# Kotstantinovskiy/SonicDiffusionBayesLab

Measured on AMD Instinct MI355X. Metric: 512x512 images/sec at 50 DDIM steps, higher is better.
Workload: dtype bf16; 1 GPU; SD-1.5 512x512 DDIM 50 steps, CFG 7.5, batch=8/GPU (BASELINE configs[1]); global_batch=8, sample_size=64, parallelism=batch-shard x1, weights=SD-1.5-shaped synthetic seed 1234

## Files before the change

include/sd_hip.h:

```cpp
#ifndef SD_HIP_H
#define SD_HIP_H

#ifdef __cplusplus
extern "C" {
#endif

typedef struct sd_unet sd_unet;

typedef struct sd_unet_config {
    int sample_size;
    int in_channels;
    int out_channels;
    int num_levels;
    int block_out_channels[8];
    int layers_per_block;
    int attn_levels[8];
    int cross_attention_dim;
    int num_heads;
    int norm_num_groups;
    float norm_eps;
    int context_len;
    int weight_dtype;
    float fp8_act_scale_norm;
    float fp8_act_scale_ff;
// ... 106 lines not shown
int sd_clip_encode(sd_clip* c, void* stream, const int* input_ids, int batch, float* hidden_out, void* workspace,
                   long long workspace_bytes);

typedef struct sd_clip_vision_config {
    int hidden_size;
    int num_layers;
    int num_heads;
    int intermediate_size;
    int image_size;
    int patch_size;
    int projection_dim;
    float layer_norm_eps;
    int hidden_act;
} sd_clip_vision_config;
enum { SD_ACT_QUICK_GELU = 0, SD_ACT_GELU = 1 };
typedef struct sd_unet sd_clip_vision;
int sd_clip_create_projected(const sd_clip_config* cfg, int projection_dim, int eos_token_id, sd_clip** out);
long long sd_clip_text_embeds_workspace_bytes(sd_clip* c, int batch);
int sd_clip_text_embeds(sd_clip* c, void* stream, const int* input_ids, int batch, float* text_embeds, void* workspace,
                        long long workspace_bytes);
int sd_clip_vision_create(const sd_clip_vision_config* cfg, sd_clip_vision** out);
long long sd_clip_vision_workspace_bytes(sd_clip_vision* v, int batch, int height, int width);
int sd_clip_vision_encode(sd_clip_vision* v, void* stream, const unsigned char* images, int batch, int height, int width,
                          float* image_embeds, void* workspace, long long workspace_bytes);
int sd_clip_score(void* stream, const float* image_embeds, const float* text_embeds, int batch, int dim, float* raw,
                  float* score);
typedef struct sd_image_reward_config {
    int vision_hidden_size;
    int vision_num_layers;
    int vision_num_heads;
    int vision_intermediate_size;
    int image_size;
    int patch_size;
    float vision_layer_norm_eps;
    int vocab_size;
    int hidden_size;
    int num_layers;
    int num_heads;
    int intermediate_size;
    int max_positions;
    float layer_norm_eps;
    int hidden_act;
    int position_embedding_absolute;
    int max_text_len;
    float reward_mean, reward_std;
} sd_image_reward_config;
typedef struct sd_unet sd_image_reward;
int sd_image_reward_create(const sd_image_reward_config* cfg, sd_image_reward** out);
long long sd_image_reward_workspace_bytes(sd_image_reward* m, int batch, int height, int width);
int sd_image_reward_score(sd_image_reward* m, void* stream, const unsigned char* images, const int* input_ids,
                          const int* attention_mask, int batch, int text_len, int height, int width, float* rewards,
                          float* features_or_null, void* workspace, long long workspace_bytes);
int sd_clip_resize_taps(int in_size, int out_size, int first, int count, int* xmin, int* xcnt, int* coeffs);

typedef struct sd_inception sd_inception;
int sd_inception_create(sd_inception** out);
void sd_inception_destroy(sd_inception* h);
int sd_inception_num_convs(const sd_inception* h);
int sd_inception_conv_info(const sd_inception* h, int index, char* name, int name_cap, long long shape[4]);
int sd_inception_load_conv(sd_inception* h, const char* name, const float* weight_oihw, long long weight_numel,
                           const float* bias, int cout);
int sd_inception_finalize(sd_inception* h);
long long sd_inception_workspace_bytes(sd_inception* h, int batch, int tap);
int sd_inception_features(sd_inception* h, void* stream, const unsigned char* images, int batch, int height, int width,
                          int tap, float* features, void* workspace, long long workspace_bytes);
int sd_fid_accumulate(void* stream, const float* features, int batch, int dim, double* sum, double* cov_sum,
                      long long* count);
int sd_op_inception_conv(void* stream, const void* X, const void* W, const float* bias, void* Y, int B, int Hin, int Win,
                         int Cin, int Cout, int kh, int kw, int stride, int pad_h, int pad_w, int ldy, int coff, int relu);
int sd_op_maxpool3x3(void* stream, const void* X, void* Y, int B, int H, int W, int C, int stride, int pad, int ldy, int coff);
int sd_op_avgpool3x3(void* stream, const void* X, void* Y, int B, int H, int W, int C, int ldy, int coff);
int sd_op_global_mean(void* stream, const void* X, float* out, int B, int HW, int C);
int sd_op_inception_resize(void* stream, const unsigned char* images, int B, int H, int W, void* out, int out_fp32);

#define SD_PROFILE_KINDS 32
int sd_unet_forward_profiled(sd_unet* u, void* stream, const float* latents, int latent_batch, int unet_batch,
                             float timestep, float* eps_out, void* workspace, long long workspace_bytes, int cache_mode,
                             int cache_branch_id, double kind_ms[SD_PROFILE_KINDS], long long kind_launches[SD_PROFILE_KINDS],
                             double kind_flops[SD_PROFILE_KINDS], double kind_bytes[SD_PROFILE_KINDS]);

long long sd_unet_forward_op_times(sd_unet* u, void* stream, const float* latents, int latent_batch, int unet_batch,
                                   float timestep, float* eps_out, void* workspace, long long workspace_bytes, int cache_mode,
                                   int cache_branch_id, char* text, long long cap);

int sd_unet_debug_tensor(sd_unet* u, void* stream, const char* name, float* host_out, long long numel,
                         void* workspace, int unet_batch, int cache_branch_id);

int sd_sched_step(void* stream, const float* eps, int cfg, float guidance, const float* x, const float* m1,
                  const float* m2, const float* m3, const float* noise, float* prev, float* y2, float* m_out,
                  const float coef[10], long long n);

int sd_cfg_rescale_factors(void* stream, const float* eps, int batch, long long n_per_sample, float guidance,
                           float rescale, float* k_out);
int sd_sched_step_rescaled(void* stream, const float* eps, int cfg, float guidance, const float* x, const float* m1,
                           const float* m2, const float* m3, const float* noise, float* prev, float* y2, float* m_out,
                           const float coef[10], long long n, const float* k, long long n_per_sample);

int sd_sched_step_inpaint(void* stream, const float* eps, int cfg, float guidance, const float* x, const float* m1,
                          const float* m2, const float* m3, const float* noise, float* prev, float* y2, float* m_out,
                          const float coef[10], long long n, const float* k, long long n_per_sample, const float* init,
                          const float* blend_noise, const float* mask, float a, float s, long long hw);
int sd_inpaint_prepare(void* stream, const float* image, const float* mask, float* masked_image, float* latent_mask,
                       int batch, int height, int width);

int sd_op_gemm(void* stream, const void* X, long long ldx, const void* X2, long long ldx2, int K1, const void* W,
               const float* bias, const float* bias2, const void* R, long long ldr, void* C, long long ldc, int M,
               int N, int K, int epi);
int sd_op_gemm_tile_rows(int M, int N, int K);
int sd_op_gemm_splitk(int M, int N, int K, int dtype);
int sd_op_gemm_batched(void* stream, const void* X, long long ldx, const void* W, long long w_batch_stride,
                       int rows_per_batch, const float* bias, const void* R, long long ldr, void* C, long long ldc,
                       int M, int N, int K, int epi, int sm_valid);
int sd_op_gemm_batched_softmax_ln(void* stream, const void* X, long long ldx, const void* W, long long w_batch_stride,
                                  int rows_per_batch, void* C, long long ldc, int M, int N, int K, int sm_valid,
                                  const float* rowstats, int parts, const float* c1, const float* c2, float eps);
int sd_op_conv3x3(void* stream, const void* X, const void* W, const float* bias, const float* bias2, const void* R,
                  void* Y, int B, int Hin, int Win, int Cin, int Cout, int stride, int upsample);
int sd_op_conv3x3_shortcut(void* stream, const void* X, const void* W, const float* bias, const void* Xs1, int Cs1,
                           const void* Xs2, int Cs2, const void* Wsc, void* Y, int B, int H, int Wd, int Cin, int Cout);
int sd_op_conv3x3_shortcut_groupnorm(void* stream, const void* X, const void* W, const float* bias, const void* Xs1, int Cs1,
                                     const void* Xs2, int Cs2, const void* Wsc, void* Y, int B, int H, int Wd, int Cin,
                                     int Cout, const float* gamma, const float* beta, void* Yn, int groups, float eps, int silu);
int sd_op_conv3x3_down_asym(void* stream, const void* X, const void* W, const float* bias, void* Y, int B, int Hin, int Win,
                            int Cin, int Cout);
int sd_op_conv3x3_kernel(int M, int N, int Cin, int Hin, int Win, int stride, int upsample, int dtype);
int sd_op_softmax_rows(void* stream, void* S, long long rows, int cols, float scale);
int sd_op_conv3x3_upsample_subpixel(void* stream, const void* X, const void* W4, const float* bias, void* Y, int B, int Hin,
                                    int Win, int Cin, int Cout);
int sd_op_conv3x3_upsample_subpixel_groupnorm(void* stream, const void* X, const void* W4, const float* bias, void* Y, int B,
                                              int Hin, int Win, int Cin, int Cout, const float* gamma, const float* beta,
                                              void* Yn, int groups, float eps, int silu);
int sd_op_groupnorm(void* stream, const void* x1, int C1, const void* x2, int C2, const float* gamma,
                    const float* beta, void* y, int B, int HW, int groups, float eps, int silu);
int sd_op_conv3x3_groupnorm(void* stream, const void* X, const void* W, const float* bias, const float* bias2,
                            const void* R, void* Y, int B, int Hin, int Win, int Cin, int Cout, const float* gamma,
                            const float* beta, void* Yn, int groups, float eps, int silu);
int sd_op_conv3x3_splitk(int M, int Cout, int Cin, int Hin, int Win, int stride, int upsample);
int sd_op_layernorm(void* stream, const void* x, const float* gamma, const float* beta, void* y, int rows, int C,
                    float eps);
int sd_op_tome_match(void* stream, const void* x, const unsigned char* choice, int B, int h, int w, int C, float* node_max,
                     int* node_idx, int* tok);
int sd_op_tome_select(void* stream, const float* node_max, const int* node_idx, int B, int num_src, int r, int* kept, int* merged,
                      int* dst_idx);
int sd_op_tome_merge(void* stream, const void* x, const int* tok, const int* kept, const int* merged, const int* dst_idx, void* out,
                     long long ldo, int B, int h, int w, int C, int r);
int sd_op_tome_unmerge(void* stream, const void* y, long long ldy, const void* residual, const int* tok, const int* kept,
                       const int* merged, const int* dst_idx, void* out, int B, int h, int w, int C, int r);
int sd_op_attention(void* stream, const void* Q, long long ldq, const void* K, long long ldk, const void* V,
                    long long ldv, void* O, long long ldo, int B, int heads, int Nq, int Nk, int D, float scale);
int sd_op_gemm_qkv_headmajor(void* stream, const void* X, long long ldx, const void* W, void* Q, void* KV, int M, int C,
                             int tokens, int K);
int sd_op_attention_headmajor(void* stream, const void* Q, long long ldq, const void* K, const void* V, void* O,
                              long long ldo, int B, int heads, int Nq, int Nk, int D, float scale);
int sd_op_clip_attention(void* stream, const void* qkv, void* out, int B, int L, int H, int heads);
int sd_op_vit_attention(void* stream, const void* qkv, void* out, int B, int L, int H, int heads);
int sd_op_bert_attention(void* stream, const void* q, long long ldq, const void* k, const void* v, long long ldkv,
                         const int* mask, void* out, long long ldo, int B, int heads, int Lq, int Lk);
int sd_op_reward_head(void* stream, const void* hidden, long long row_stride, const float* w, const float* bias, float mean,
                      float std, int B, int H, float* rewards, float* features);
int sd_op_clip_preprocess(void* stream, const unsigned char* images, int B, int H, int W, int S, int P, unsigned char* crop,
                          void* patches);
int sd_op_conv_in(void* stream, const float* x, int Bsrc, const float* Wt, const float* bias, void* y, int B, int H,
                  int W, int Cin, int Cout);
int sd_op_conv_in_cond(void* stream, const float* x, int Bsrc, const float* cond, int Bcond, const float* Wt,
                       const float* bias, void* y, int B, int H, int W, int Cout);
int sd_op_conv_in_add(void* stream, const float* x, int Bsrc, const void* addend, int Badd, const float* Wt, const float* bias,
                      void* y, int B, int H, int W, int Cout);
int sd_op_residual_add(void* stream, void* x, const long long* dst_off, const void* r, const long long* src_off,
                       const long long* count, int nseg, float scale);
int sd_op_conv_out(void* stream, const void* x, const void* Wp, const float* bias, float* y, int B, int H, int W,
                   int Cin, int Cout);
int sd_op_time_embedding(void* stream, float t, const void* W1, const float* b1, const void* W2, const float* b2,
                         float* scratch, float* temb, int dim_in, int dim);
int sd_op_timestep_cond(void* stream, float t, const float* cond, const void* Wc, float* row, float* emb, int cond_dim,
                        int dim);

int sd_op_ln_partials(int kind, int M, int N);
int sd_op_gemm_rowstats(void* stream, const void* X, long long ldx, const void* W, const float* bias, const void* R,
                        long long ldr, void* C, long long ldc, int M, int N, int K, float* rowstats);
int sd_op_gemm_ln(void* stream, const void* X, long long ldx, const void* Wg, const float* c1, const float* c2,
                  const float* rowstats, int parts, float eps, void* C, long long ldc, int M, int N, int K, int epi);
int sd_op_gemm_plan(void* stream, const void* X, long long ldx, const void* X2, long long ldx2, int K1, const void* W,
                    const float* bias, const float* bias2, const void* R, long long ldr, void* C, long long ldc, int M, int N,
                    int K, float* rowstats, float* stats, const float* ln_rs, int ln_parts, const float* ln_c1, float ln_eps,
                    void* KV, int hm_tokens);
int sd_op_xattn_fused_rowstats(void* stream, const void* X, const void* R, void* Y, const void* At, const void* Bw,
                               const float* bias, int M, int C, int rows_per_sample, int L, float* rowstats);
int sd_op_ip_xattn(void* stream, const void* R, void* Rout, const void* A, const void* Bt, const float* gamma, const float* beta,
                   float eps, long long M, int C, int rows_per_sample, int heads, int T);
int sd_op_xattn_fused(void* stream, const void* X, const void* R, void* Y, const void* At, const void* Bw,
                      const float* bias, int M, int C, int rows_per_sample, int L);
int sd_op_xattn_fused_ln(void* stream, const void* X, const void* R, void* Y, const void* At, const void* Bw,
                         const float* bias, int M, int C, int rows_per_sample, int L, const float* ln_rowstats, int ln_parts,
                         long long ln_rows, const float* c2, float eps, float* rowstats);
int sd_op_conv3x3_ablate(void* stream, const void* X, const void* W, void* Y, int B, int Hin, int Win, int Cin, int Cout,
                         int ablate);
int sd_op_xattn_fused_stamps(void* stream, const void* X, const void* R, void* Y, const void* At, const void* Bw,
                             const float* bias, int M, int C, int rows_per_sample, int L, unsigned long long* stamps);

int sd_op_gemm_fp8(void* stream, const void* X, long long ldx, const void* W, const float* wscale, float xscale,
                   const float* bias, const void* R, long long ldr, void* C, long long ldc, int M, int N, int K, int epi,
                   int out_fp8, float oscale);
int sd_op_conv3x3_fp8(void* stream, const void* X, const void* W, const float* wscale, float xscale, const float* bias,
                      const float* bias2, const void* R, void* Y, int B, int Hin, int Win, int Cin, int Cout, int stride,
                      int upsample);
int sd_op_groupnorm_fp8(void* stream, const void* x1, int C1, const void* x2, int C2, const float* gamma,
                        const float* beta, void* y, int B, int HW, int groups, float eps, int silu, int Cpad, float oscale);
int sd_op_layernorm_fp8(void* stream, const void* x, const float* gamma, const float* beta, void* y, int rows, int C,
                        int Cpad, float eps, float oscale);
int sd_op_quantize_fp8(void* stream, const void* x_bf16, void* y_fp8, long long rows, int C, int Cpad, float scale);
int sd_op_amax_e4m3(void* stream, const void* codes, long long nbytes, unsigned* out_code);

#ifdef __cplusplus
}
#endif
#endif
```

sonicdiffusionbayeslab_amd/_lib.py:

```python
from __future__ import annotations

import ctypes as C
import os
import re
from typing import Optional

HERE = os.path.dirname(os.path.abspath(__file__))
LIB_PATH = os.environ.get("SD_AMD_LIB", os.path.join(HERE, "lib", "libsdhip.so"))
HEADER_PATH = os.path.normpath(os.path.join(HERE, "..", "include", "sd_hip.h"))

ABLATE_LIB_PATH = os.path.join(HERE, "lib", "libsdhip_ablate.so")

_lib: Optional[C.CDLL] = None
_ablate: Optional[C.CDLL] = None


class SdUnetConfig(C.Structure):
    _fields_ = [
        ("sample_size", C.c_int), ("in_channels", C.c_int), ("out_channels", C.c_int),
        ("num_levels", C.c_int), ("block_out_channels", C.c_int * 8), ("layers_per_block", C.c_int),
        ("attn_levels", C.c_int * 8), ("cross_attention_dim", C.c_int), ("num_heads", C.c_int),
        ("norm_num_groups", C.c_int), ("norm_eps", C.c_float), ("context_len", C.c_int),
        ("weight_dtype", C.c_int), ("fp8_act_scale_norm", C.c_float), ("fp8_act_scale_ff", C.c_float),
        ("time_cond_proj_dim", C.c_int),
# ... 38 lines not shown
    ]


class SdHipError(RuntimeError):
    pass


def declared_symbols() -> list:
    src = open(HEADER_PATH).read()
    src = re.sub(r"/\*.*?\*/", "", src, flags=re.S)
    return sorted(set(re.findall(r"\b(sd_[a-z0-9_]+)\s*\(", src)))


_vp, _i, _ll, _f = C.c_void_p, C.c_int, C.c_longlong, C.c_float
_SIGS = {
    "sd_last_error": (C.c_char_p, []),
    "sd_abi_version": (_i, []),
    "sd_unet_create": (_i, [C.POINTER(SdUnetConfigFull), C.POINTER(_vp)]),
    "sd_unet_destroy": (None, [_vp]),
    "sd_unet_num_params": (_i, [_vp]),
    "sd_unet_param_info": (_i, [_vp, _i, C.c_char_p, _i, C.POINTER(_ll), C.POINTER(_i)]),
    "sd_unet_load_param": (_i, [_vp, C.c_char_p, _vp, _ll]),
    "sd_unet_finalize": (_i, [_vp]),
    "sd_unet_debug_packed": (_ll, [_vp, C.c_char_p, _vp, _ll]),
    "sd_unet_calibrate_fp8": (_i, [_vp, _vp, _vp, _i, _i, _f, _f, _vp, _ll]),
    "sd_unet_fp8_scale_count": (_i, [_vp]),
    "sd_unet_fp8_scale_info": (_i, [_vp, _i, C.c_char_p, _i, C.POINTER(_f), C.POINTER(_f)]),
    "sd_unet_set_fp8_scale": (_i, [_vp, C.c_char_p, _f]),
    "sd_unet_workspace_bytes": (_ll, [_vp, _i, _i]),
    "sd_unet_set_context": (_i, [_vp, _vp, _vp, _i, _i, _vp, _ll]),
    "sd_unet_set_timestep_cond": (_i, [_vp, _vp, _vp]),
    "sd_unet_forward": (_i, [_vp, _vp, _vp, _i, _i, _f, _vp, _vp, _ll, _i, _i]),
    "sd_unet_workspace_bytes_hw": (_ll, [_vp, _i, _i, _i, _i]),
    "sd_unet_set_context_hw": (_i, [_vp, _vp, _vp, _i, _i, _i, _i, _vp, _ll]),
    "sd_unet_forward_hw": (_i, [_vp, _vp, _vp, _i, _i, _i, _i, _f, _vp, _vp, _ll, _i, _i]),
    "sd_unet_forward_profiled": (_i, [_vp, _vp, _vp, _i, _i, _f, _vp, _vp, _ll, _i, _i, C.POINTER(C.c_double),
                                      C.POINTER(_ll), C.POINTER(C.c_double), C.POINTER(C.c_double)]),
    "sd_unet_forward_op_times": (_ll, [_vp, _vp, _vp, _i, _i, _f, _vp, _vp, _ll, _i, _i, C.c_char_p, _ll]),
    "sd_vae_create": (_i, [C.POINTER(SdUnetConfigFull), C.POINTER(_vp)]),
    "sd_vae_decode": (_i, [_vp, _vp, _vp, _i, _f, _vp, _vp, _ll]),
    "sd_vae_decode_hw": (_i, [_vp, _vp, _vp, _i, _i, _i, _f, _vp, _vp, _ll]),
    "sd_vae_encoder_create": (_i, [C.POINTER(SdUnetConfigFull), C.POINTER(_vp)]),
    "sd_vae_encode_hw": (_i, [_vp, _vp, _vp, _i, _i, _i, _vp, _vp, _ll]),
    "sd_vae_posterior_sample": (_i, [_vp, _vp, _vp, _f, _vp, _i, _ll]),
    "sd_taesd_decoder_create": (_i, [C.POINTER(_vp)]),
    "sd_taesd_encoder_create": (_i, [C.POINTER(_vp)]),
    "sd_taesd_decode_hw": (_i, [_vp, _vp, _vp, _i, _i, _i, _i, _vp, _vp, _ll]),
    "sd_taesd_encode_hw": (_i, [_vp, _vp, _vp, _i, _i, _i, _vp, _vp, _ll]),
    "sd_op_conv64": (_i, [_vp, _vp, _vp, _vp, _vp, _vp, _i, _i, _i, _i, _i]),
    "sd_op_conv64_pack": (_ll, [_vp, _vp]),
    "sd_op_taesd_entry": (_i, [_vp, _vp, _vp, _vp, _vp, _i, _i, _i, _i, _i]),
    "sd_op_taesd_exit": (_i, [_vp, _vp, _vp, _vp, _vp, _i, _i, _i, _i, _i]),
    "sd_clip_create": (_i, [C.POINTER(SdClipConfig), C.POINTER(_vp)]),
    "sd_clip_encode": (_i, [_vp, _vp, _vp, _i, _vp, _vp, _ll]),
    "sd_clip_create_projected": (_i, [C.POINTER(SdClipConfig), _i, _i, C.POINTER(_vp)]),
    "sd_clip_text_embeds_workspace_bytes": (_ll, [_vp, _i]),
    "sd_clip_text_embeds": (_i, [_vp, _vp, _vp, _i, _vp, _vp, _ll]),
    "sd_clip_vision_create": (_i, [C.POINTER(SdClipVisionConfig), C.POINTER(_vp)]),
    "sd_clip_vision_workspace_bytes": (_ll, [_vp, _i, _i, _i]),
    "sd_clip_vision_encode": (_i, [_vp, _vp, _vp, _i, _i, _i, _vp, _vp, _ll]),
    "sd_clip_score": (_i, [_vp, _vp, _vp, _i, _i, _vp, _vp]),
    "sd_image_reward_create": (_i, [C.POINTER(SdImageRewardConfig), C.POINTER(_vp)]),
    "sd_image_reward_workspace_bytes": (_ll, [_vp, _i, _i, _i]),
    "sd_image_reward_score": (_i, [_vp, _vp, _vp, _vp, _vp, _i, _i, _i, _i, _vp, _vp, _vp, _ll]),
    "sd_op_bert_attention": (_i, [_vp, _vp, _ll, _vp, _vp, _ll, _vp, _vp, _ll, _i, _i, _i, _i]),
    "sd_op_reward_head": (_i, [_vp, _vp, _ll, _vp, _vp, _f, _f, _i, _i, _vp, _vp]),
    "sd_clip_resize_taps": (_i, [_i, _i, _i, _i, _vp, _vp, _vp]),
    "sd_op_vit_attention": (_i, [_vp, _vp, _vp, _i, _i, _i, _i]),
    "sd_op_clip_preprocess": (_i, [_vp, _vp, _i, _i, _i, _i, _i, _vp, _vp]),
    "sd_inception_create": (_i, [C.POINTER(_vp)]),
    "sd_inception_destroy": (None, [_vp]),
    "sd_inception_num_convs": (_i, [_vp]),
    "sd_inception_conv_info": (_i, [_vp, _i, C.c_char_p, _i, C.POINTER(_ll)]),
    "sd_inception_load_conv": (_i, [_vp, C.c_char_p, _vp, _ll, _vp, _i]),
    "sd_inception_finalize": (_i, [_vp]),
    "sd_inception_workspace_bytes": (_ll, [_vp, _i, _i]),
    "sd_inception_features": (_i, [_vp, _vp, _vp, _i, _i, _i, _i, _vp, _vp, _ll]),
    "sd_fid_accumulate": (_i, [_vp, _vp, _i, _i, _vp, _vp, _vp]),
    "sd_op_inception_conv": (_i, [_vp, _vp, _vp, _vp, _vp, _i, _i, _i, _i, _i, _i, _i, _i, _i, _i, _i, _i, _i]),
    "sd_op_maxpool3x3": (_i, [_vp, _vp, _vp, _i, _i, _i, _i, _i, _i, _i, _i]),
    "sd_op_avgpool3x3": (_i, [_vp, _vp, _vp, _i, _i, _i, _i, _i, _i]),
    "sd_op_global_mean": (_i, [_vp, _vp, _vp, _i, _i, _i]),
    "sd_op_inception_resize": (_i, [_vp, _vp, _i, _i, _i, _vp, _i]),
    "sd_unet_debug_tensor": (_i, [_vp, _vp, C.c_char_p, _vp, _ll, _vp, _i, _i]),
    "sd_sched_step": (_i, [_vp, _vp, _i, _f, _vp, _vp, _vp, _vp, _vp, _vp, _vp, _vp, C.POINTER(_f), _ll]),
    "sd_cfg_rescale_factors": (_i, [_vp, _vp, _i, _ll, _f, _f, _vp]),
    "sd_sched_step_rescaled": (_i, [_vp, _vp, _i, _f, _vp, _vp, _vp, _vp, _vp, _vp, _vp, _vp, C.POINTER(_f), _ll, _vp, _ll]),
    "sd_sched_step_inpaint": (_i, [_vp, _vp, _i, _f, _vp, _vp, _vp, _vp, _vp, _vp, _vp, _vp, C.POINTER(_f), _ll, _vp, _ll,
                                   _vp, _vp, _vp, _f, _f, _ll]),
    "sd_inpaint_prepare": (_i, [_vp, _vp, _vp, _vp, _vp, _i, _i, _i]),
    "sd_unet_set_inpaint_cond_hw": (_i, [_vp, _vp, _vp, _vp, _i, _i, _i]),
    "sd_unet_set_ip_adapter_hw": (_i, [_vp, _vp, _vp, _i, _i, _i, _i, _f, _vp, _ll]),
    "sd_op_ip_xattn": (_i, [_vp, _vp, _vp, _vp, _vp, _vp, _vp, _f, _ll, _i, _i, _i, _i]),
    "sd_controlnet_create": (_i, [C.POINTER(SdUnetConfigFull), C.POINTER(_i), C.POINTER(_vp)]),
    "sd_controlnet_residual_bytes_hw": (_ll, [_vp, _i, _i, _i]),
    "sd_controlnet_set_cond_hw": (_i, [_vp, _vp, _vp, _i, _i, _i]),
    "sd_controlnet_forward_hw": (_i, [_vp, _vp, _vp, _i, _i, _i, _i, _f, _vp, _vp, _ll]),
    "sd_unet_set_control_residuals_hw": (_i, [_vp, _vp, _f, _i, _i, _i]),
    "sd_op_conv_in_add": (_i, [_vp, _vp, _i, _vp, _i, _vp, _vp, _vp, _i, _i, _i, _i]),
    "sd_op_residual_add": (_i, [_vp, _vp, _vp, _vp, _vp, _vp, _i, _f]),
    "sd_op_conv_in_cond": (_i, [_vp, _vp, _i, _vp, _i, _vp, _vp, _vp, _i, _i, _i, _i]),
    "sd_op_gemm": (_i, [_vp, _vp, _ll, _vp, _ll, _i, _vp, _vp, _vp, _vp, _ll, _vp, _ll, _i, _i, _i, _i]),
    "sd_op_gemm_tile_rows": (_i, [_i, _i, _i]),
    "sd_op_gemm_splitk": (_i, [_i, _i, _i, _i]),
    "sd_op_gemm_batched": (_i, [_vp, _vp, _ll, _vp, _ll, _i, _vp, _vp, _ll, _vp, _ll, _i, _i, _i, _i, _i]),
    "sd_op_gemm_batched_softmax_ln": (_i, [_vp, _vp, _ll, _vp, _ll, _i, _vp, _ll, _i, _i, _i, _i, _vp, _i, _vp, _vp, _f]),
    "sd_op_conv3x3": (_i, [_vp, _vp, _vp, _vp, _vp, _vp, _vp, _i, _i, _i, _i, _i, _i, _i]),
    "sd_op_conv3x3_shortcut": (_i, [_vp, _vp, _vp, _vp, _vp, _i, _vp, _i, _vp, _vp, _i, _i, _i, _i, _i]),
    "sd_op_conv3x3_shortcut_groupnorm": (_i, [_vp, _vp, _vp, _vp, _vp, _i, _vp, _i, _vp, _vp, _i, _i, _i, _i, _i,
                                              _vp, _vp, _vp, _i, _f, _i]),
    "sd_op_conv3x3_down_asym": (_i, [_vp, _vp, _vp, _vp, _vp, _i, _i, _i, _i, _i]),
    "sd_op_conv3x3_ablate": (_i, [_vp, _vp, _vp, _vp, _i, _i, _i, _i, _i, _i]),
    "sd_op_conv3x3_upsample_subpixel": (_i, [_vp, _vp, _vp, _vp, _vp, _i, _i, _i, _i, _i]),
    "sd_op_conv3x3_upsample_subpixel_groupnorm": (_i, [_vp, _vp, _vp, _vp, _vp, _i, _i, _i, _i, _i, _vp, _vp, _vp, _i, _f, _i]),
    "sd_op_groupnorm": (_i, [_vp, _vp, _i, _vp, _i, _vp, _vp, _vp, _i, _i, _i, _f, _i]),
    "sd_op_conv3x3_groupnorm": (_i, [_vp, _vp, _vp, _vp, _vp, _vp, _vp, _i, _i, _i, _i, _i, _vp, _vp, _vp, _i, _f, _i]),
    "sd_op_conv3x3_splitk": (_i, [_i, _i, _i, _i, _i, _i, _i]),
    "sd_op_conv3x3_kernel": (_i, [_i, _i, _i, _i, _i, _i, _i, _i]),
    "sd_op_softmax_rows": (_i, [_vp, _vp, _ll, _i, _f]),
    "sd_op_layernorm": (_i, [_vp, _vp, _vp, _vp, _vp, _i, _i, _f]),
    "sd_op_attention": (_i, [_vp, _vp, _ll, _vp, _ll, _vp, _ll, _vp, _ll, _i, _i, _i, _i, _i, _f]),
    "sd_op_gemm_qkv_headmajor": (_i, [_vp, _vp, _ll, _vp, _vp, _vp, _i, _i, _i, _i]),
    "sd_op_attention_headmajor": (_i, [_vp, _vp, _ll, _vp, _vp, _vp, _ll, _i, _i, _i, _i, _i, _f]),
    "sd_op_clip_attention": (_i, [_vp, _vp, _vp, _i, _i, _i, _i]),
    "sd_op_conv_in": (_i, [_vp, _vp, _i, _vp, _vp, _vp, _i, _i, _i, _i, _i]),
    "sd_op_conv_out": (_i, [_vp, _vp, _vp, _vp, _vp, _i, _i, _i, _i, _i]),
    "sd_op_time_embedding": (_i, [_vp, _f, _vp, _vp, _vp, _vp, _vp, _vp, _i, _i]),
    "sd_op_timestep_cond": (_i, [_vp, _f, _vp, _vp, _vp, _vp, _i, _i]),
    "sd_op_ln_partials": (_i, [_i, _i, _i]),
    "sd_op_gemm_rowstats": (_i, [_vp, _vp, _ll, _vp, _vp, _vp, _ll, _vp, _ll, _i, _i, _i, _vp]),
    "sd_op_gemm_plan": (_i, [_vp, _vp, _ll, _vp, _ll, _i, _vp, _vp, _vp, _vp, _ll, _vp, _ll, _i, _i, _i, _vp, _vp, _vp, _i, _vp, _f,
                            _vp, _i]),
    "sd_op_gemm_ln": (_i, [_vp, _vp, _ll, _vp, _vp, _vp, _vp, _i, _f, _vp, _ll, _i, _i, _i, _i]),
    "sd_op_xattn_fused_rowstats": (_i, [_vp, _vp, _vp, _vp, _vp, _vp, _vp, _i, _i, _i, _i, _vp]),
    "sd_op_xattn_fused": (_i, [_vp, _vp, _vp, _vp, _vp, _vp, _vp, _i, _i, _i, _i]),
    "sd_op_xattn_fused_ln": (_i, [_vp, _vp, _vp, _vp, _vp, _vp, _vp, _i, _i, _i, _i, _vp, _i, _ll, _vp, _f, _vp]),
    "sd_op_xattn_fused_stamps": (_i, [_vp, _vp, _vp, _vp, _vp, _vp, _vp, _i, _i, _i, _i, _vp]),
    "sd_op_gemm_fp8": (_i, [_vp, _vp, _ll, _vp, _vp, _f, _vp, _vp, _ll, _vp, _ll, _i, _i, _i, _i, _i, _f]),
    "sd_op_conv3x3_fp8": (_i, [_vp, _vp, _vp, _vp, _f, _vp, _vp, _vp, _vp, _i, _i, _i, _i, _i, _i, _i]),
    "sd_op_groupnorm_fp8": (_i, [_vp, _vp, _i, _vp, _i, _vp, _vp, _vp, _i, _i, _i, _f, _i, _i, _f]),
    "sd_op_layernorm_fp8": (_i, [_vp, _vp, _vp, _vp, _vp, _i, _i, _i, _f, _f]),
    "sd_op_quantize_fp8": (_i, [_vp, _vp, _vp, _ll, _i, _i, _f]),
    "sd_op_amax_e4m3": (_i, [_vp, _vp, _ll, _vp]),
    "sd_unet_set_tome": (_i, [_vp, C.c_double, _i]),
    "sd_unet_tome_block_count_hw": (_i, [_vp, _i, _i]),
    "sd_unet_tome_block_info_hw": (_i, [_vp, _i, _i, _i, C.POINTER(_i), C.POINTER(_i), C.POINTER(_i), C.POINTER(_ll)]),
    "sd_unet_set_tome_choice_hw": (_i, [_vp, _vp, _vp, _ll, _i, _i]),
    "sd_unet_tome_matching_hw": (_i, [_vp, _vp, _i, _i, _i, _vp, _vp, _vp, _vp, _vp, C.POINTER(_i), C.POINTER(_i)]),
    "sd_op_tome_match": (_i, [_vp, _vp, _vp, _i, _i, _i, _i, _vp, _vp, _vp]),
    "sd_op_tome_select": (_i, [_vp, _vp, _vp, _i, _i, _i, _vp, _vp, _vp]),
    "sd_op_tome_merge": (_i, [_vp, _vp, _vp, _vp, _vp, _vp, _vp, _ll, _i, _i, _i, _i, _i]),
    "sd_op_tome_unmerge": (_i, [_vp, _vp, _ll, _vp, _vp, _vp, _vp, _vp, _vp, _i, _i, _i, _i, _i]),
}


def load() -> C.CDLL:
    global _lib
    if _lib is not None:
        return _lib
    if not os.path.exists(LIB_PATH):
        raise SdHipError(
            f"{LIB_PATH} is missing: build it with `python -m sonicdiffusionbayeslab_amd.build` "
            "(or __graft_entry__.build()).  There is no CPU/PyTorch fallback for the hot path.")
    lib = C.CDLL(LIB_PATH)
    for name, (res, args) in _SIGS.items():
        fn = getattr(lib, name)
        fn.restype = res
        fn.argtypes = args
    _lib = lib
    return lib


def load_ablate() -> C.CDLL:
    global _ablate
    if _ablate is not None:
        return _ablate
    if not os.path.exists(ABLATE_LIB_PATH):
        raise SdHipError(f"{ABLATE_LIB_PATH} is missing: build it with `python -m sonicdiffusionbayeslab_amd.build`")
    lib = C.CDLL(ABLATE_LIB_PATH)
    for name, (res, args) in _SIGS.items():
        fn = getattr(lib, name)
        fn.restype = res
        fn.argtypes = args
    _ablate = lib
    return lib


def check(rc: int, what: str = "libsdhip call", lib: Optional[C.CDLL] = None) -> None:
    if rc != 0:
        msg = (lib or load()).sd_last_error()
        raise SdHipError(f"{what} failed (rc={rc}): {msg.decode() if msg else '?'}")


def ptr(t) -> Optional[int]:
    return None if t is None else t.data_ptr()


def current_stream() -> int:
    import torch
    return torch.cuda.current_stream().cuda_stream
```

sonicdiffusionbayeslab_amd/csrc/gemm_conv.hip:

```cpp
#include "common.h"
#include "kernels.h"

#include <stdlib.h>

#ifdef SD_ABLATE
#define SD_TUNE(p) ((p).tune)
#else
#define SD_TUNE(p) 0
#endif

namespace {

constexpr int AMODE_GEMM = 0;
constexpr int AMODE_CONV = 1;
constexpr int EPI_STD = 0;
constexpr int EPI_GEGLU = 1;
constexpr int EPI_SOFTMAX = 2;

constexpr int kPersistentGrid = 512;

template <int N>
__device__ __forceinline__ void wait_vmcnt() {
    asm volatile("s_waitcnt vmcnt(%0)" ::"n"(N) : "memory");
}
// ... 580 lines not shown
    GemmArgs a = a0;
    a.tiles_m = (a.M + BM - 1) / BM;
    a.tiles_n = (a.N + BN - 1) / BN;
    if (a.ldw == 0) a.ldw = a.K;
    if (EPI != EPI_STD || a.slab == nullptr || a.splitk < 1) a.splitk = 1;
    SD_REQUIRE(!a.defer_reduce || a.splitk > 1, "gemm: defer_reduce needs split-K (the consumer would read an unwritten slab)");
#ifdef SD_ABLATE
    static const int tune = getenv("SD_GEMM_TUNE") ? atoi(getenv("SD_GEMM_TUNE")) : 0;
    a.tune = tune;
#else
    a.tune = 0;
#endif
    constexpr int smem = STAGES * (BM + BN) * 128 + (STAGES == 2 && DT == 0 ? WAVES_M * WAVES_N * 512 + 2 * BN * 4 : 0);
    static_assert(smem <= 160 * 1024, "tile does not fit the 160 KiB LDS");
    auto kern = gemm_kernel<BM, BN, WAVES_M, WAVES_N, STAGES, AMODE, EPI, DT>;
    static bool attr_set = false;
    if (!attr_set) {
        SD_CHECK_HIP(hipFuncSetAttribute((const void*)kern, hipFuncAttributeMaxDynamicSharedMemorySize, smem));
        attr_set = true;
    }
    int grid = a.tiles_m * a.tiles_n * a.splitk;
    constexpr int persistent = smem > 80 * 1024 ? kPersistentGrid / 2 : kPersistentGrid;
    if (STAGES == 2 && grid > persistent) grid = persistent;
    hipLaunchKernelGGL(kern, dim3(grid), dim3(WAVES_M * WAVES_N * 64), smem, stream, a);
    if (a.splitk > 1 && !a.defer_reduce) sd_launch_splitk_reduce(a, stream);
    SD_CHECK_HIP(hipGetLastError());
    return 0;
}

}

void sd_launch_splitk_reduce(const GemmArgs& a, hipStream_t stream) {
    const long n4 = (long)a.M * (a.N / 4);
    hipLaunchKernelGGL(splitk_reduce_kernel, dim3((unsigned)((n4 + 255) / 256)), dim3(256), 0, stream, a);
}

static int big_tile_mode() {
    static const char* env = getenv("SD_GEMM_BIG");
    return env ? atoi(env) : 0;
}
static bool big_tile_ok(int M, int N, int BN) {
    (void)M; (void)N; (void)BN;
    return big_tile_mode() == 1;
}

int sd_gemm_tile_rows(int M, int N, int K) {
    static const bool off = getenv("SD_GEMM_SMALL") && atoi(getenv("SD_GEMM_SMALL")) == 0;
    if (K >= 4096 && M >= 4096) return 128;
    return (!off && M > 64 && ((M + 127) / 128) * ((N + 159) / 160) < 384) ? 64 : 128;
}

int sd_gemm_splitk(int M, int N, int K, int rows) {
    static const char* env = getenv("SD_SPLITK");
    if (env) return atoi(env) > 1 ? atoi(env) : 1;
    if (rows == 0) rows = sd_gemm_tile_rows(M, N, K);
    const int tiles = ((M + rows - 1) / rows) * ((N + 159) / 160);
    const int KT = K / 64;
    if (tiles >= 448) return 1;
    int want = (512 + tiles - 1) / tiles;
    int maxs = KT / 12;
    int s = want < maxs ? want : maxs;
    if (s > 8) s = 8;
    return s < 1 ? 1 : s;
}

static int check_fp8(const GemmArgs& a, const char* what) {
    SD_REQUIRE(a.wscale != nullptr && a.xscale_inv > 0.f, "%s fp8: weight scales / activation scale missing", what);
    SD_REQUIRE(a.K % 128 == 0 && a.K >= 128, "%s fp8: K=%d must be a positive multiple of 128", what, a.K);
    SD_REQUIRE(a.X2 == nullptr && a.K1 == a.K, "%s fp8: no second K segment", what);
    SD_REQUIRE(a.rows_per_batch == 0, "%s fp8: per-sample weights are bf16 only", what);
    SD_REQUIRE(((uintptr_t)a.X & 15) == 0 && ((uintptr_t)a.W & 15) == 0, "%s fp8: operands must be 16-byte aligned", what);
    return 0;
}

static int check_stats(const GemmArgs& a, int epi) {
    if (!a.stats) return 0;
    SD_REQUIRE(epi == EPI_STD && a.M % 64 == 0 && !(a.splitk > 1 && a.slab) && !a.out_fp8,
               "producer statistics: plain epilogue, M %% 64 == 0 and no split-K (M=%d splitk=%d)", a.M, a.splitk);
    return 0;
}
static int check_headmajor(const GemmArgs& a, int epi) {
    if (!a.hm_C) return 0;
    SD_REQUIRE(epi == EPI_STD && a.KV && a.hm_C % 160 == 0 && a.N == 3 * a.hm_C && a.hm_tok % 128 == 0 && a.M % a.hm_tok == 0 &&
                   !(a.splitk > 1 && a.slab) && big_tile_mode() == 0 && sd_gemm_tile_rows(a.M, a.N) == 128,
               "head-major K / V: N = 3 C with C %% 160 == 0, tokens per sample %% 128 == 0, 128 x 160 tiles, no split-K");
    return 0;
}
static int check_ln(const GemmArgs& a, int epi) {
    if (a.rowstats) SD_REQUIRE(epi == EPI_STD && !(a.splitk > 1 && a.slab), "LayerNorm partials: plain epilogue without split-K");
    if (!a.ln_rs) return 0;
    SD_REQUIRE((epi == EPI_STD || epi == EPI_GEGLU || epi == EPI_SOFTMAX) && a.dt == 0 && !(a.splitk > 1 && a.slab) && a.ln_c1 && a.ln_np > 0 &&
               a.ln_np <= 16 && a.X2 == nullptr && a.K1 == a.K && a.K >= 128 && big_tile_mode() == 0 && a.bias && !a.R && !a.bias2,
               "LayerNorm fold: bf16 operands, std / GEGLU epilogue, one K segment, no split-K (epi=%d np=%d)", epi, a.ln_np);
    return 0;
}

int sd_launch_gemm(const GemmArgs& a, int epi, hipStream_t stream) {
    if (check_stats(a, epi) || check_ln(a, epi) || check_headmajor(a, epi)) return -1;
    if (a.dt == 1) {
        if (check_fp8(a, "gemm")) return -1;
        SD_REQUIRE(a.N % 4 == 0 && a.M > 0 && a.N > 0 && a.zero_page, "gemm fp8: bad problem");
        SD_REQUIRE(a.ldx % 16 == 0 && (a.ldw == 0 || a.ldw % 16 == 0), "gemm fp8: row strides must be multiples of 16 bytes");
        if (epi == EPI_GEGLU) {
            SD_REQUIRE(a.N % 32 == 0, "geglu gemm: N=%d must be a multiple of 32", a.N);
            SD_REQUIRE(!a.out_fp8 || (a.ldc % 4 == 0), "geglu gemm fp8 out: ldc=%ld must be a multiple of 4 bytes", a.ldc);
            if (a.N % 256 == 0) return launch<256, 256, 4, 2, 2, AMODE_GEMM, EPI_GEGLU, 1>(a, stream);
            return launch<128, 128, 2, 2, 2, AMODE_GEMM, EPI_GEGLU, 1>(a, stream);
        }
        SD_REQUIRE(epi == EPI_STD && !a.out_fp8, "gemm fp8: epilogue %d not built", epi);
        return launch<128, 160, 2, 2, 2, AMODE_GEMM, EPI_STD, 1>(a, stream);
    }
    SD_REQUIRE(!a.out_fp8, "gemm: fp8 output needs fp8 operands");
    SD_REQUIRE(a.K % 64 == 0 && a.K >= 64, "gemm: K=%d must be a positive multiple of 64", a.K);
    SD_REQUIRE(a.N % 4 == 0, "gemm: N=%d must be a multiple of 4", a.N);
    SD_REQUIRE(a.K1 % 64 == 0 && a.K1 <= a.K, "gemm: K1=%d must be a multiple of 64 and <= K", a.K1);
    SD_REQUIRE(a.K1 == a.K || a.X2 != nullptr, "gemm: second K segment needs X2");
    SD_REQUIRE(a.M > 0 && a.N > 0, "gemm: empty problem");
    SD_REQUIRE(a.zero_page != nullptr, "gemm: zero page missing");
    const char* lean_env = getenv("SD_GEMM_LEAN");
    const bool lean_off = lean_env && atoi(lean_env) == 0;
    if (epi == EPI_GEGLU) {
        SD_REQUIRE(a.N % 32 == 0, "geglu gemm: N=%d must be a multiple of 32", a.N);
        if (!lean_off && big_tile_mode() == 0 && sd_gemm_lean_applicable(a, 1)) return sd_launch_gemm_lean(a, 1, 256, stream);
        if (big_tile_ok(a.M, a.N, 128)) return launch<256, 128, 4, 2, 3, AMODE_GEMM, EPI_GEGLU>(a, stream);
        if (big_tile_mode() != 3 && a.N % 256 == 0) return launch<256, 256, 4, 2, 2, AMODE_GEMM, EPI_GEGLU>(a, stream);
        return launch<128, 128, 2, 2, 2, AMODE_GEMM, EPI_GEGLU>(a, stream);
    }
    SD_REQUIRE(a.rows_per_batch == 0 || a.rows_per_batch % 128 == 0,
               "gemm: rows_per_batch=%d must be a multiple of the 128-row tile", a.rows_per_batch);
    if (epi == EPI_SOFTMAX) {
        SD_REQUIRE(a.N % 80 == 0 && a.sm_valid > 0 && a.sm_valid <= 80 && a.R == nullptr && (a.bias == nullptr || a.ln_rs),
                   "softmax gemm: N=%d must be a multiple of 80, 0 < sm_valid=%d <= 80, no bias/residual", a.N, a.sm_valid);
        SD_REQUIRE(!a.ln_per_sample || (a.ln_rs && a.rows_per_batch > 0), "gemm: per-sample LayerNorm vectors need per-sample weights");
        return launch<128, 160, 2, 2, 2, AMODE_GEMM, EPI_SOFTMAX>(a, stream);
    }
    if (a.rows_per_batch) return launch<128, 160, 2, 2, 2, AMODE_GEMM, EPI_STD>(a, stream);
    if (!lean_off && big_tile_mode() == 0 && sd_gemm_lean_applicable(a, epi)) {
        const int rows = (!a.stats && !a.ln_rs && !a.hm_C) ? sd_gemm_tile_rows(a.M, a.N, a.K) : 128;
        return sd_launch_gemm_lean(a, 0, rows, stream);
    }
    if (big_tile_ok(a.M, a.N, 160)) return launch<256, 160, 4, 2, 3, AMODE_GEMM, EPI_STD>(a, stream);
    if (big_tile_mode() == 2) return launch<256, 160, 4, 2, 2, AMODE_GEMM, EPI_STD>(a, stream);
    if (!a.stats && !a.ln_rs && sd_gemm_tile_rows(a.M, a.N, a.K) == 64) return launch<64, 160, 2, 2, 2, AMODE_GEMM, EPI_STD>(a, stream);
    return launch<128, 160, 2, 2, 2, AMODE_GEMM, EPI_STD>(a, stream);
}

int sd_launch_conv3x3(const GemmArgs& a, hipStream_t stream) {
    if (check_stats(a, EPI_STD)) return -1;
    if (a.dt == 1) {
        if (check_fp8(a, "conv3x3")) return -1;
        SD_REQUIRE(a.Cin % 128 == 0, "conv3x3 fp8: Cin=%d must be a multiple of 128 (pad the channels)", a.Cin);
    }
    SD_REQUIRE(a.Cin % 64 == 0, "conv3x3: Cin=%d must be a multiple of 64", a.Cin);
    if (a.subpix) {
        SD_REQUIRE(a.dt == 0 && a.K == 4 * a.Cin && a.N % 4 == 0 && a.Hout == 2 * a.Hin && a.Wout == 2 * a.Win && a.stride == 1 &&
                       a.up == 0 && (a.Hin * a.Win) % 64 == 0 && a.M % (4 * a.Hin * a.Win) == 0 && a.R == nullptr &&
                       a.zero_page != nullptr && a.w_batch_stride > 0 && !(a.splitk > 1 && a.slab),
                   "conv3x3 sub-pixel upsample: bf16, K = 4 Cin, low-res pixels per sample %% 64 == 0, no residual, no split-K");
        if (sd_conv_halo_subpix_applicable(a)) return sd_launch_conv3x3_halo(a, stream);
        if ((a.Hin * a.Win) % 128 != 0) {
            SD_REQUIRE(!a.stats, "conv3x3 sub-pixel upsample: block statistics need low-res pixels per sample %% 128 == 0");
            return launch<64, 160, 2, 2, 2, AMODE_CONV, EPI_STD>(a, stream);
        }
        return launch<128, 160, 2, 2, 2, AMODE_CONV, EPI_STD>(a, stream);
    }
    SD_REQUIRE(a.K == 9 * a.Cin, "conv3x3: K must be 9*Cin");
    SD_REQUIRE(a.N % 4 == 0, "conv3x3: Cout=%d must be a multiple of 4", a.N);
    SD_REQUIRE(a.stride == 1 || a.stride == 2, "conv3x3: stride %d", a.stride);
    SD_REQUIRE(!(a.up && a.stride != 1), "conv3x3: upsample needs stride 1");
    SD_REQUIRE(a.zero_page != nullptr, "conv3x3: zero page missing");
    const int hv = a.Hin << a.up, wv = a.Win << a.up;
    SD_REQUIRE(!a.asym || (a.stride == 2 && a.dt == 0 && a.Hin % 2 == 0 && a.Win % 2 == 0 && !a.stats),
               "conv3x3: the asymmetric form is bf16, stride 2, even input sides (%dx%d stride %d)", a.Hin, a.Win, a.stride);
    SD_REQUIRE(a.Hout == (hv + 2 - 3) / a.stride + 1 && a.Wout == (wv + 2 - 3) / a.stride + 1,
               "conv3x3: output size %dx%d inconsistent with input %dx%d stride %d up %d", a.Hout, a.Wout,
               a.Hin, a.Win, a.stride, a.up);
    SD_REQUIRE(a.M % (a.Hout * a.Wout) == 0, "conv3x3: M not a multiple of Hout*Wout");
    SD_REQUIRE(!a.Wsc || sd_conv_halo_shortcut_applicable(a), "conv3x3: the 1x1 shortcut (%d + %d channels) cannot ride on this conv",
               a.Csc1, a.Csc2);
    if (sd_conv_halo_applicable(a)) return sd_launch_conv3x3_halo(a, stream);
    if (a.dt == 1) return launch<128, 160, 2, 2, 2, AMODE_CONV, EPI_STD, 1>(a, stream);
    if (big_tile_ok(a.M, a.N, 160)) return launch<256, 160, 4, 2, 3, AMODE_CONV, EPI_STD>(a, stream);
    return launch<128, 160, 2, 2, 2, AMODE_CONV, EPI_STD>(a, stream);
}
```

sonicdiffusionbayeslab_amd/csrc/gemm_lean.hip:

```cpp
#include "common.h"
#include "kernels.h"
#include <mutex>
#include <stdlib.h>

namespace {

typedef __amdgpu_buffer_rsrc_t rsrc_t;

struct LeanArgs {
    const void* X; const void* X2; const void* W; const void* R; void* C; void* KV;
    const float* vec0; const float* vec1;
    const float* ln_rs; float* rowstats; float* stats;
    unsigned x_bytes, x2_bytes, w_bytes, r_bytes, c_bytes, kv_bytes;
    int M, N, K, K1;
    int ldxb, ldx2b, ldwb, ldrb, ldcb;
    int tiles_m, tiles_n;
    float ln_eps, inv_k;
    int hm_tpc;
    int hm_tok_shift, hm_heads, hm_samples;
};

template <int N>
__device__ __forceinline__ void wait_vmcnt() {
    asm volatile("s_waitcnt vmcnt(%0)" ::"n"(N) : "memory");
// ... 254 lines not shown
                    *(f32x4*)(dst + a * 128) = f32x4{sv[0], qv[0], sv[1], qv[1]};
                    *(f32x4*)(dst + a * 128 + 16) = f32x4{sv[2], qv[2], sv[3], qv[3]};
                }
            }
        }
        if (!LN && !GEGLU && p.rowstats) {
            char* dst = (char*)p.rowstats + ((long)(etile_n * WAVES_N + wn) * p.M + em0) * 8 + (unsigned)vRs;
#pragma unroll
            for (int b = 0; b < TM; ++b) {
                float s = 0.f, q = 0.f;
#pragma unroll
                for (int a = 0; a < TN; ++a) {
                    const unsigned p0 = pack2bf(acc[a][b][0], acc[a][b][1]), p1 = pack2bf(acc[a][b][2], acc[a][b][3]);
                    const float v[4] = {bflo(p0), bfhi(p0), bflo(p1), bfhi(p1)};
#pragma unroll
                    for (int j = 0; j < 4; ++j) { s += v[j]; q = __builtin_fmaf(v[j], v[j], q); }
                }
                s += __shfl_xor(s, 16); q += __shfl_xor(q, 16);
                s += __shfl_xor(s, 32); q += __shfl_xor(q, 32);
                if (lq == 0) *(f32x2_t*)(dst + b * 16 * 8) = f32x2_t{s, q};
            }
        }
        if constexpr (GEGLU) {
            auto geglu_tile = [&](int a, int b) -> u32x2 {
                const f32x4 va = acc[a][b], vg = acc[a + 1][b];
                const f32x2_t lo = geglu_pair(f32x2_t{va[0], va[1]}, f32x2_t{vg[0], vg[1]});
                const f32x2_t hi = geglu_pair(f32x2_t{va[2], va[3]}, f32x2_t{vg[2], vg[3]});
                return u32x2{pack2bf(lo[0], lo[1]), pack2bf(hi[0], hi[1])};
            };
            const int soC = em0 * p.ldcb + en0;
#pragma unroll
            for (int b = 0; b < TM; ++b) {
                const int vo = vCg + (soC + b * 16 * p.ldcb);
#pragma unroll
                for (int a = 0; a < TN; a += 4) {
                    const u32x2 ox = geglu_tile(a, b), oy = geglu_tile(a + 2, b);
                    const auto s0 = __builtin_amdgcn_permlane16_swap(ox[0], oy[0], false, false);
                    const auto s1 = __builtin_amdgcn_permlane16_swap(ox[1], oy[1], false, false);
                    __builtin_amdgcn_raw_buffer_store_b128(u32x4{s0[0], s1[0], s0[1], s1[1]}, rC, vo + a * 16, 0, 0);
                }
            }
        } else {
            u32x4 ow[TM][TN / 2];
            u32x2 on[TM];
#pragma unroll
            for (int b = 0; b < TM; ++b) {
#pragma unroll
                for (int a = 0; a + 1 < TN; a += 2) {
                    const f32x4 vx = acc[a][b], vy = acc[a + 1][b];
                    const auto s0 = __builtin_amdgcn_permlane16_swap(pack2bf(vx[0], vx[1]), pack2bf(vy[0], vy[1]), false, false);
                    const auto s1 = __builtin_amdgcn_permlane16_swap(pack2bf(vx[2], vx[3]), pack2bf(vy[2], vy[3]), false, false);
                    ow[b][a / 2] = u32x4{s0[0], s1[0], s0[1], s1[1]};
                }
                const f32x4 v = acc[TN - 1][b];
                on[b] = u32x2{pack2bf(v[0], v[1]), pack2bf(v[2], v[3])};
            }
            if (LN && p.hm_tpc > 0 && etile_n >= p.hm_tpc) {
                const int which = etile_n >= 2 * p.hm_tpc ? 1 : 0;
                const int head0 = (etile_n - (which + 1) * p.hm_tpc) * 4;
                const int smp = em0 >> p.hm_tok_shift, tok0 = em0 & ((1 << p.hm_tok_shift) - 1);
                const int soC = ((((which * p.hm_samples + smp) * p.hm_heads + head0) << p.hm_tok_shift) + tok0) * 80;
#pragma unroll
                for (int b = 0; b < TM; ++b) {
                    const int so = soC + b * 16 * 80;
#pragma unroll
                    for (int j = 0; j < TN / 2; ++j) __builtin_amdgcn_raw_buffer_store_b128(ow[b][j], rKV, vH[j] + so, 0, 0);
                    __builtin_amdgcn_raw_buffer_store_b64(on[b], rKV, vH[TN / 2] + so, 0, 0);
                }
            } else {
                const int soC = em0 * p.ldcb + en0 * 2;
#pragma unroll
                for (int b = 0; b < TM; ++b) {
                    const int so = soC + b * 16 * p.ldcb;
#pragma unroll
                    for (int j = 0; j < TN / 2; ++j) __builtin_amdgcn_raw_buffer_store_b128(ow[b][j], rC, vCw + so + j * 64, 0, 0);
                    __builtin_amdgcn_raw_buffer_store_b64(on[b], rC, vCn + so + (TN - 1) * 32, 0, 0);
                }
            }
        }
        if (!more) break;
    }
}

static const float* zero_vector() {
    static std::mutex mu;
    static float* z[16] = {};
    int dev = 0;
    if (hipGetDevice(&dev) != hipSuccess || dev < 0 || dev >= 16) return nullptr;
    std::lock_guard<std::mutex> lock(mu);
    if (!z[dev]) {
        float* p = nullptr;
        float probe = 1.f;
        if (hipMalloc((void**)&p, 16384 * 4) != hipSuccess) return nullptr;
        if (hipMemset(p, 0, 16384 * 4) != hipSuccess || hipMemcpy(&probe, p + 16383, 4, hipMemcpyDeviceToHost) != hipSuccess || probe != 0.f) {
            (void)hipFree(p);
            return nullptr;
        }
        z[dev] = p;
    }
    return z[dev];
}

template <int BM, int BN, int WAVES_M, int WAVES_N, int NP, bool GEGLU>
int launch_lean(const LeanArgs& a0, hipStream_t stream) {
    LeanArgs a = a0;
    a.tiles_m = (a.M + BM - 1) / BM;
    a.tiles_n = a.N / BN;
    constexpr int NW = WAVES_M * WAVES_N;
    constexpr int smem = 2 * (BM + BN) * 128 + NW * 512 + 2 * BN * 4;
    static_assert(smem <= 160 * 1024, "tile does not fit the 160 KiB LDS");
    auto kern = gemm_lean_kernel<BM, BN, WAVES_M, WAVES_N, NP, GEGLU>;
    static bool attr_set = false;
    if (!attr_set) {
        SD_CHECK_HIP(hipFuncSetAttribute((const void*)kern, hipFuncAttributeMaxDynamicSharedMemorySize, smem));
        attr_set = true;
    }
    int grid = a.tiles_m * a.tiles_n;
    constexpr int resident = smem > 80 * 1024 ? 256 : 512;
    if (grid > resident) grid = resident;
    hipLaunchKernelGGL(kern, dim3(grid), dim3(NW * 64), smem, stream, a);
    SD_CHECK_HIP(hipGetLastError());
    return 0;
}

}

bool sd_gemm_lean_applicable(const GemmArgs& a, int epi) {
    if ((epi != 0 && epi != 1) || a.dt != 0 || a.out_fp8 || a.rows_per_batch || a.subpix || (a.splitk > 1 && a.slab)) return false;
    const int BN = epi ? 256 : 160;
    if (a.N % BN != 0 || a.N > 16384 || a.K % 64 != 0 || a.K < 128 || a.K1 % 64 != 0 || a.M < 1) return false;
    if (a.K1 != a.K && a.X2 == nullptr) return false;
    if ((a.ldc & 7) || (a.ldx & 7) || (a.X2 && (a.ldx2 & 7)) || (a.ldw & 7) || (a.R && (a.ldr & 3))) return false;
    const long big = 1L << 31;
    const long ldw = a.ldw ? a.ldw : a.K;
    if ((long)a.M * a.ldx * 2 >= big || (long)a.M * a.ldc * 2 >= big || (long)a.N * ldw * 2 >= big) return false;
    if (a.X2 && (long)a.M * a.ldx2 * 2 >= big) return false;
    if (a.R && (long)a.M * a.ldr * 2 >= big) return false;
    if ((a.stats || a.rowstats || a.ln_rs || a.hm_C) && a.M % (epi ? 256 : 128) != 0) return false;
    if (a.ln_rs) {
        if (a.R || a.bias2 || !a.bias || !a.ln_c1 || a.X2 || a.K1 != a.K || a.stats || a.rowstats) return false;
        if (a.ln_np != 2 && a.ln_np != 4 && a.ln_np != 8 && a.ln_np != 16) return false;
    }
    if (epi == 1 && (a.R || a.bias2 || a.X2 || a.K1 != a.K || a.stats || a.rowstats || a.hm_C)) return false;
    if (a.hm_C) {
        if (!a.ln_rs || !a.KV || a.hm_C % 160 != 0 || a.N != 3 * a.hm_C || a.hm_tok < 128 || (a.hm_tok & (a.hm_tok - 1)) ||
            a.M % a.hm_tok != 0 || (long)a.M * a.hm_C * 4 >= big)
            return false;
    }
    return true;
}

int sd_launch_gemm_lean(const GemmArgs& g, int epi, int rows, hipStream_t stream) {
    SD_REQUIRE(sd_gemm_lean_applicable(g, epi), "gemm (lean): problem not supported (M=%d N=%d K=%d epi=%d)", g.M, g.N, g.K, epi);
    SD_REQUIRE(epi == 1 || rows == 128 || (rows == 64 && !g.stats && !g.ln_rs && !g.hm_C),
               "gemm (lean): %d-row tile with block statistics / LayerNorm fold / head-major K|V", rows);
    const long ldw = g.ldw ? g.ldw : g.K;
    LeanArgs a{};
    a.X = g.X; a.X2 = g.X2; a.W = g.W; a.R = g.R; a.C = g.C; a.KV = g.KV;
    a.M = g.M; a.N = g.N; a.K = g.K; a.K1 = g.K1;
    a.ldxb = (int)g.ldx * 2; a.ldx2b = (int)g.ldx2 * 2; a.ldwb = (int)ldw * 2; a.ldrb = (int)g.ldr * 2; a.ldcb = (int)g.ldc * 2;
    a.x_bytes = (unsigned)(((long)g.M - 1) * g.ldx * 2 + (long)g.K1 * 2);
    a.x2_bytes = g.X2 ? (unsigned)(((long)g.M - 1) * g.ldx2 * 2 + (long)(g.K - g.K1) * 2) : 0;
    a.w_bytes = (unsigned)(((long)g.N - 1) * ldw * 2 + (long)g.K * 2);
    a.r_bytes = g.R ? (unsigned)(((long)g.M - 1) * g.ldr * 2 + (long)g.N * 2) : 0;
    const int ncols = epi ? g.N / 2 : g.hm_C ? g.hm_C : g.N;
    a.c_bytes = (unsigned)(((long)g.M - 1) * g.ldc * 2 + (long)ncols * 2);
    a.kv_bytes = g.hm_C ? (unsigned)((long)g.M * g.hm_C * 4) : 0;
    const float* zeros = nullptr;
    if (!g.bias || (!g.ln_rs && !g.bias2)) {
        zeros = zero_vector();
        SD_REQUIRE(zeros, "gemm (lean): cannot allocate the zero vector");
    }
    if (g.ln_rs) {
        a.vec0 = g.ln_c1; a.vec1 = g.bias; a.ln_rs = g.ln_rs; a.ln_eps = g.ln_eps; a.inv_k = 1.0f / (float)g.K;
    } else {
        a.vec0 = g.bias ? g.bias : zeros; a.vec1 = g.bias2 ? g.bias2 : zeros;
    }
    a.rowstats = g.rowstats; a.stats = g.stats;
    if (g.hm_C) {
        a.hm_tpc = g.hm_C / 160;
        int sh = 0;
        while ((1 << sh) < g.hm_tok) ++sh;
        a.hm_tok_shift = sh; a.hm_heads = g.hm_C / 40; a.hm_samples = g.M / g.hm_tok;
    }
    if (epi == 1) {
        if (!g.ln_rs) return launch_lean<256, 256, 4, 2, 0, true>(a, stream);
        return g.ln_np == 2 ? launch_lean<256, 256, 4, 2, 2, true>(a, stream)
             : g.ln_np == 4 ? launch_lean<256, 256, 4, 2, 4, true>(a, stream)
             : g.ln_np == 8 ? launch_lean<256, 256, 4, 2, 8, true>(a, stream) : launch_lean<256, 256, 4, 2, 16, true>(a, stream);
    }
    if (g.ln_rs)
        return g.ln_np == 2 ? launch_lean<128, 160, 2, 2, 2, false>(a, stream)
             : g.ln_np == 4 ? launch_lean<128, 160, 2, 2, 4, false>(a, stream)
             : g.ln_np == 8 ? launch_lean<128, 160, 2, 2, 8, false>(a, stream) : launch_lean<128, 160, 2, 2, 16, false>(a, stream);
    return rows == 64 ? launch_lean<64, 160, 2, 2, 0, false>(a, stream) : launch_lean<128, 160, 2, 2, 0, false>(a, stream);
}
```

sonicdiffusionbayeslab_amd/csrc/kernels.h:

```cpp
#pragma once
#include <vector>

#include "common.h"

struct GemmArgs {
    const bf16_t* X = nullptr;
    long ldx = 0;
    const bf16_t* X2 = nullptr;
    long ldx2 = 0;
    int K1 = 0;
    const bf16_t* W = nullptr;
    long ldw = 0;
    const float* bias = nullptr;
    const float* bias2 = nullptr;
    const bf16_t* R = nullptr;
    long ldr = 0;
    bf16_t* C = nullptr;
    long ldc = 0;
    int M = 0, N = 0, K = 0;
    int Hin = 0, Win = 0, Cin = 0, Hout = 0, Wout = 0, stride = 1, up = 0;
    int asym = 0;
    int splitk = 1;
    float* slab = nullptr;
    int defer_reduce = 0;
    const void* zero_page = nullptr;
    long w_batch_stride = 0;
    int rows_per_batch = 0;
    int sm_valid = 0;
    int tiles_m = 0, tiles_n = 0;
    int tune = 0;
    float* stats = nullptr;
    float* rowstats = nullptr;
    bf16_t* KV = nullptr;
    int hm_C = 0, hm_tok = 0;
    int subpix = 0;
    const float* ln_rs = nullptr;
    const float* ln_c1 = nullptr;
    int ln_np = 0;
    float ln_eps = 1e-5f;
    int ln_per_sample = 0;
    int dt = 0;
    const float* wscale = nullptr;
    float xscale_inv = 1.0f;
    int out_fp8 = 0;
    float oscale = 1.0f;
    const bf16_t* Xs1 = nullptr;
    const bf16_t* Xs2 = nullptr;
    const bf16_t* Wsc = nullptr;
    long ldwsc = 0;
    int Csc1 = 0, Csc2 = 0;
};

int sd_gemm_tile_rows(int M, int N, int K = 0);
int sd_gemm_splitk(int M, int N, int K, int rows = 0);
int sd_launch_gemm(const GemmArgs& a, int epi , hipStream_t stream);
int sd_launch_conv3x3(const GemmArgs& a, hipStream_t stream);
bool sd_gemm_lean_applicable(const GemmArgs& a, int epi);
int sd_launch_gemm_lean(const GemmArgs& a, int epi, int rows, hipStream_t stream);
void sd_launch_splitk_reduce(const GemmArgs& a, hipStream_t stream);
bool sd_conv_halo_applicable(const GemmArgs& a);
int sd_conv_halo_mode(const GemmArgs& a);
int sd_conv3x3_splitk(int M, int N, int Cin, int Hin, int Win, int stride, int up, int dt = 0);
bool sd_conv_halo_subpix_applicable(const GemmArgs& a);
int sd_launch_conv3x3_halo(const GemmArgs& a, hipStream_t stream);
bool sd_conv_halo_shortcut_applicable(const GemmArgs& a);

constexpr int SD_CONV64_PACKED_BYTES = 9 * 2 * 4 * 1024;
struct Conv64Args {
    const bf16_t* X = nullptr;
    const bf16_t* Wp = nullptr;
    const float* bias = nullptr;
    const bf16_t* R = nullptr;
    bf16_t* Y = nullptr;
    int B = 0, Hin = 0, Win = 0;
    int mode = 0;
    int relu = 0;
    int Hout = 0, Wout = 0, tiles_y = 0, tiles_x = 0, ntiles = 0;
    unsigned xbytes = 0;
};
int sd_conv64_out_size(int in, int mode);
void sd_conv64_pack(const float* w_oihw , bf16_t* out);
int sd_launch_conv64(const Conv64Args& a, hipStream_t stream);
int sd_launch_taesd_entry(const float* x, const float* Wt, const float* bias, bf16_t* y, int B, int H, int W, int Cin, int decoder,
                          hipStream_t stream);
int sd_launch_taesd_exit(const bf16_t* x, const bf16_t* Wp, const float* bias, float* y, int B, int H, int W, int Cout, int out_mode,
                         hipStream_t stream);

struct GroupNormArgs {
    const bf16_t* x1 = nullptr; int C1 = 0;
    const bf16_t* x2 = nullptr; int C2 = 0;
    const float* gamma = nullptr; const float* beta = nullptr;
    bf16_t* y = nullptr;
    int out_fp8 = 0, Cpad = 0;
    float oscale = 1.0f;
    const float* stats1 = nullptr; const float* stats2 = nullptr;
    const float* slab = nullptr; int splitk = 0;
    const float* sbias = nullptr; const float* sbias2 = nullptr;
    const bf16_t* sR = nullptr; long sldr = 0;
    bf16_t* x1w = nullptr;
    float* partial = nullptr;
    int B = 0, HW = 0, groups = 32, nsplit = 0;
    float eps = 1e-5f;
    int silu = 0;
};
int sd_groupnorm_nsplit(int B, int HW);
bool sd_groupnorm_uses_small(int B, int HW, int C1, int C2, int groups);
bool sd_groupnorm_slab_ok(int B, int HW, int C1, int C2, int groups);
size_t sd_groupnorm_scratch_bytes(int B, int HW, int groups);
int sd_launch_groupnorm(const GroupNormArgs& a, hipStream_t stream);

int sd_launch_softmax_rows(bf16_t* s, long rows, int cols, float scale, hipStream_t stream);
int sd_launch_softmax_rows_long(bf16_t* s, long rows, int cols, float scale, hipStream_t stream);
int sd_launch_pqconv(const float* x, const float* W, const float* bias, float* y, int B, int HW, float in_scale,
                     hipStream_t stream);

int sd_launch_layernorm(const bf16_t* x, const float* gamma, const float* beta, bf16_t* y, int rows, int C,
                        float eps, hipStream_t stream);
int sd_launch_layernorm_fp8(const bf16_t* x, const float* gamma, const float* beta, void* y, int rows, int C, int Cpad,
                            float eps, float oscale, hipStream_t stream);
int sd_launch_amax_e4m3(const void* y, long nbytes, unsigned* out, hipStream_t stream);
int sd_launch_quantize_fp8(const bf16_t* x, void* y, long rows, int C, int Cpad, float scale, hipStream_t stream);

struct AttnArgs {
    const bf16_t* Q = nullptr; long ldq = 0;
    const bf16_t* K = nullptr; long ldk = 0;
    const bf16_t* V = nullptr; long ldv = 0;
    bf16_t* O = nullptr; long ldo = 0;
    int B = 0, heads = 0, Nq = 0, Nk = 0, D = 0;
    float scale = 0.f;
    const void* consts = nullptr;
    int kv_head_major = 0;
    int q_prescaled = 0;
    int xcd_order = 1;
};
int sd_launch_attention(const AttnArgs& a, hipStream_t stream);

int sd_launch_gemv(const float* x, const bf16_t* W, const float* b, float* y, int N, int K, int silu_in,
                   hipStream_t stream);
int sd_launch_timestep_sinusoid(float t, float* out, int dim, hipStream_t stream);
int sd_launch_timestep_sinusoid_row(float t, const float* row, float* out, int dim, hipStream_t stream);
int sd_launch_f32_to_bf16(const float* src, bf16_t* dst, long n, hipStream_t stream);
// ... 114 lines not shown
```

sonicdiffusionbayeslab_amd/csrc/model.h:

```cpp
#pragma once
#include "../../include/sd_hip.h"
#include "common.h"
#include "kernels.h"

#include <stdlib.h>
#include <string.h>
#include <sys/mman.h>

#include <algorithm>
#include <map>
#include <new>
#include <set>
#include <string>
#include <tuple>
#include <unordered_map>
#include <vector>

namespace sdhip {

constexpr size_t NOFF = (size_t)-1;
constexpr int T_LATENTS = -2, T_EPS = -3;
constexpr int MAX_CONTROL_RES = SD_MAX_RES_SEGMENTS;

struct ParamSpec {
    std::string name;
    std::vector<long long> shape;
    std::vector<float> data;
    bool loaded = false;
    long long numel() const {
        long long n = 1;
        for (auto s : shape) n *= s;
        return n;
    }
};

struct Wrap {
    int type;
    int block_i, layer_i;
};

enum OpKind { OP_SINUSOID, OP_GEMV, OP_CONV_IN, OP_GN, OP_CONV3, OP_GEMM, OP_LN, OP_ATTN, OP_CONV_OUT, OP_SOFTMAX, OP_PQCONV,
              OP_CLIP_EMBED, OP_CLIP_ATTN, OP_QGELU, OP_TO_F32, OP_XATTN, OP_REPLICATE,
              OP_VIT_PREP, OP_VIT_EMBED, OP_VIT_ATTN, OP_POOL, OP_CONV_IN_IMG, OP_ENC_OUT, OP_IP_XATTN, OP_RES_ADD,
              OP_BERT_ATTN, OP_REWARD_HEAD,
              OP_TOME_MATCH, OP_TOME_SELECT, OP_TOME_MERGE, OP_TOME_UNMERGE };

constexpr int REP_TEXT_POOLED = 2;

struct Op {
    int kind = 0;
    int x1 = -1, x2 = -1, r = -1, out = -1, aux = -1, b2t = -1;
    size_t w = NOFF, b = NOFF, g = NOFF, be = NOFF;
    long b2idx = 0;
    int M = 0, N = 0, K = 0, K1 = 0, epi = 0;
    int B = 0, Hin = 0, Win = 0, Cin = 0, Hout = 0, Wout = 0, stride = 1, up = 0;
    int C1 = 0, C2 = 0, HW = 0, silu = 0, nsplit = 0;
    float eps = 0.f;
    int heads = 0, D = 0, Nq = 0, Nk = 0;
    long ldq = 0, ldk = 0, ldv = 0, ldo = 0, qoff = 0, koff = 0, voff = 0;
    int silu_in = 0, splitk = 1;
    int pool_by_ids = 0;
    int key_mask = 0;
    int defer = 0, slab_t = -1, slab_k = 0, slab_r = -1, slab_b2t = -1;
    size_t slab_b = NOFF;
    long slab_b2idx = 0;
    int wt = -1;
    size_t wx = NOFF;
    long xoff = 0, woff_el = 0, coff = 0, ldx_o = 0, ldw_o = 0, ldc_o = 0;
    float scale = 0.f;
    long wbs = 0;
    int rpb = 0, sm_valid = 0;
    int dt = 0, out_fp8 = 0, Cpad = 0, Kalg = 0;
    int sname = -1;
    int stats = -1, s1 = -1, s2 = -1;
    int subpix = 0;
    int asym = 0;
    int hm = 0;
    int qps = 0;
    int rs = -1, lnrs = -1, lnnp = 0;
    size_t c1 = NOFF;
    size_t wsc = NOFF;
    float xs = 1.f, os = 1.f;
    int scx1 = -1, scx2 = -1, scc1 = 0, scc2 = 0;
    size_t scw = NOFF;
    int nres = 0;
    int res_t[MAX_CONTROL_RES];
    int nwrap = 0;
    Wrap wraps[3];
};

struct HostBlob {
    unsigned char* p = nullptr;
    size_t n = 0, cap = 0;
    unsigned char* data() { return p; }
    const unsigned char* data() const { return p; }
    size_t size() const { return n; }
    bool empty() const { return n == 0; }
    bool reserve(size_t bytes) {
        if (bytes <= cap) return true;
        void* q = mmap(nullptr, bytes, PROT_READ | PROT_WRITE, MAP_PRIVATE | MAP_ANONYMOUS | MAP_POPULATE, -1, 0);
        if (q == MAP_FAILED) return false;
        (void)madvise(q, bytes, MADV_HUGEPAGE);
        if (p) { memcpy(q, p, n); munmap(p, cap); }
        p = (unsigned char*)q; cap = bytes;
        return true;
    }
    void resize(size_t bytes) {
        if (bytes > cap && !reserve(std::max(bytes, cap * 2))) throw std::bad_alloc();
        n = bytes;
    }
    void release() { if (p) munmap(p, cap); p = nullptr; n = cap = 0; }
    ~HostBlob() { release(); }
    HostBlob() = default;
    HostBlob(const HostBlob&) = delete;
    HostBlob& operator=(const HostBlob&) = delete;
};

struct Tn {
    size_t bytes = 0;
    int def = -1, last = -1;
    bool persistent = false;
    bool ctx = false;
    bool ctx_ip = false;
    size_t off = NOFF;
};

struct Plan {
    int UB = 0, branch = -1;
    int rep = 1;
    int lh = 0, lw = 0;
    int ip = 0;
    struct IpFold { int at, bt, C; size_t wqT, wo, wkv; int heads; };
    std::vector<IpFold> ip_fold;
    int ip_e = -1, ip_proj = -1, ip_tok = -1, ip_kv = -1;
    int cn = 0;
    std::vector<size_t> cn_off;
    std::vector<long> cn_count;
    struct TomeBlock { int tok, kept, merged, dst_idx, B, h, w, r; long choice_off; };
    std::vector<TomeBlock> tome;
    long tome_choice_bytes = 0;
    std::vector<Tn> tensors;
    std::vector<Op> ops;
    std::vector<char> skipped;
// ... 124 lines not shown
```

sonicdiffusionbayeslab_amd/csrc/ops.hip:

```cpp
#include "model.h"

#include <stdlib.h>

namespace sdhip {

static void* g_scratch = nullptr;
static size_t g_scratch_bytes = 0;
void* op_scratch(size_t bytes) {
    if (bytes > g_scratch_bytes) {
        (void)hipDeviceSynchronize();
        if (g_scratch) (void)hipFree(g_scratch);
        g_scratch = nullptr;
        g_scratch_bytes = 0;
        if (hipMalloc(&g_scratch, bytes) != hipSuccess) return nullptr;
        g_scratch_bytes = bytes;
    }
    return g_scratch;
}

}

using namespace sdhip;

static void conv3x3_args(GemmArgs& a, const void* X, const void* W, const float* bias, const float* bias2, const void* R, void* Y,
// ... 460 lines not shown
extern "C" int sd_op_gemm_fp8(void* stream, const void* X, long long ldx, const void* W, const float* wscale, float xscale,
                              const float* bias, const void* R, long long ldr, void* C, long long ldc, int M, int N, int K,
                              int epi, int out_fp8, float oscale) {
    if (ensure_zero_page()) return -2;
    SD_REQUIRE(epi == 0 || epi == 1, "sd_op_gemm_fp8: epi %d (0 = std, 1 = GEGLU)", epi);
    SD_REQUIRE(xscale > 0.f && (!out_fp8 || (epi == 1 && oscale > 0.f)), "sd_op_gemm_fp8: bad scales / fp8 output needs the GEGLU epilogue");
    GemmArgs a;
    a.X = (const bf16_t*)X; a.ldx = ldx; a.K1 = K; a.W = (const bf16_t*)W; a.bias = bias; a.R = (const bf16_t*)R; a.ldr = ldr;
    a.C = (bf16_t*)C; a.ldc = ldc; a.M = M; a.N = N; a.K = K; a.zero_page = zero_page();
    a.dt = 1; a.wscale = wscale; a.xscale_inv = 1.0f / xscale; a.out_fp8 = out_fp8; a.oscale = oscale;
    a.splitk = epi ? 1 : op_gemm_splitk(M, N, K, 1);
    if (splitk_slab(a, "sd_op_gemm_fp8")) return -1;
    return sd_launch_gemm(a, epi, (hipStream_t)stream);
}

extern "C" int sd_op_conv3x3_fp8(void* stream, const void* X, const void* W, const float* wscale, float xscale,
                                 const float* bias, const float* bias2, const void* R, void* Y, int B, int Hin, int Win,
                                 int Cin, int Cout, int stride, int upsample) {
    if (ensure_zero_page()) return -2;
    SD_REQUIRE(stride == 1 || stride == 2, "conv3x3 fp8: stride %d", stride);
    SD_REQUIRE(xscale > 0.f, "conv3x3 fp8: activation scale");
    GemmArgs a;
    conv3x3_args(a, X, W, bias, bias2, R, Y, B, Hin, Win, Cin, Cout, stride, upsample ? 1 : 0);
    a.dt = 1; a.wscale = wscale; a.xscale_inv = 1.0f / xscale;
    a.splitk = sd_conv3x3_splitk(a.M, a.N, Cin, Hin, Win, stride, a.up, 1);
    if (splitk_slab(a, "sd_op_conv3x3_fp8")) return -1;
    return sd_launch_conv3x3(a, (hipStream_t)stream);
}

extern "C" int sd_op_groupnorm_fp8(void* stream, const void* x1, int C1, const void* x2, int C2, const float* gamma,
                                   const float* beta, void* y, int B, int HW, int groups, float eps, int silu, int Cpad,
                                   float oscale) {
    GroupNormArgs a;
    a.x1 = (const bf16_t*)x1; a.C1 = C1; a.x2 = (const bf16_t*)x2; a.C2 = C2; a.gamma = gamma; a.beta = beta;
    a.y = (bf16_t*)y; a.B = B; a.HW = HW; a.groups = groups; a.eps = eps; a.silu = silu;
    a.out_fp8 = 1; a.Cpad = Cpad; a.oscale = oscale;
    a.nsplit = sd_groupnorm_nsplit(B, HW);
    a.partial = (float*)op_scratch(sd_groupnorm_scratch_bytes(B, HW, groups));
    SD_REQUIRE(a.partial, "sd_op_groupnorm_fp8: cannot allocate scratch");
    return sd_launch_groupnorm(a, (hipStream_t)stream);
}

extern "C" int sd_op_layernorm_fp8(void* stream, const void* x, const float* gamma, const float* beta, void* y, int rows,
                                   int C, int Cpad, float eps, float oscale) {
    return sd_launch_layernorm_fp8((const bf16_t*)x, gamma, beta, y, rows, C, Cpad, eps, oscale, (hipStream_t)stream);
}

extern "C" int sd_op_quantize_fp8(void* stream, const void* x_bf16, void* y_fp8, long long rows, int C, int Cpad, float scale) {
    return sd_launch_quantize_fp8((const bf16_t*)x_bf16, y_fp8, (long)rows, C, Cpad, scale, (hipStream_t)stream);
}

extern "C" int sd_op_amax_e4m3(void* stream, const void* codes, long long nbytes, unsigned* out_code) {
    SD_REQUIRE(out_code, "sd_op_amax_e4m3: null output");
    SD_CHECK_HIP(hipMemsetAsync(out_code, 0, sizeof(unsigned), (hipStream_t)stream));
    return sd_launch_amax_e4m3(codes, (long)nbytes, out_code, (hipStream_t)stream);
}

extern "C" int sd_op_ln_partials(int kind, int M, int N) { return kind == 0 ? (N + 159) / 160 * 2 : 2 * sd_xattn_slices(M, N); }
extern "C" int sd_op_gemm_rowstats(void* stream, const void* X, long long ldx, const void* W, const float* bias, const void* R,
                                   long long ldr, void* C, long long ldc, int M, int N, int K, float* rowstats) {
    if (ensure_zero_page()) return -2;
    SD_REQUIRE(rowstats, "sd_op_gemm_rowstats: null partials buffer");
    GemmArgs a;
    a.X = (const bf16_t*)X; a.ldx = ldx; a.K1 = K; a.W = (const bf16_t*)W; a.bias = bias; a.R = (const bf16_t*)R; a.ldr = ldr;
    a.C = (bf16_t*)C; a.ldc = ldc; a.M = M; a.N = N; a.K = K; a.zero_page = zero_page(); a.splitk = 1; a.rowstats = rowstats;
    return sd_launch_gemm(a, 0, (hipStream_t)stream);
}
extern "C" int sd_op_gemm_plan(void* stream, const void* X, long long ldx, const void* X2, long long ldx2, int K1, const void* W,
                               const float* bias, const float* bias2, const void* R, long long ldr, void* C, long long ldc,
                               int M, int N, int K, float* rowstats, float* stats, const float* ln_rs, int ln_parts,
                               const float* ln_c1, float ln_eps, void* KV, int hm_tokens) {
    if (ensure_zero_page()) return -2;
    GemmArgs a;
    a.X = (const bf16_t*)X; a.ldx = ldx; a.X2 = (const bf16_t*)X2; a.ldx2 = ldx2; a.K1 = K1; a.W = (const bf16_t*)W;
    a.bias = bias; a.bias2 = bias2; a.R = (const bf16_t*)R; a.ldr = ldr; a.C = (bf16_t*)C; a.ldc = ldc; a.M = M; a.N = N; a.K = K;
    a.zero_page = zero_page(); a.splitk = 1; a.rowstats = rowstats; a.stats = stats;
    a.ln_rs = ln_rs; a.ln_np = ln_parts; a.ln_c1 = ln_c1; a.ln_eps = ln_eps;
    if (hm_tokens > 0) {
        SD_REQUIRE(N % 3 == 0 && KV, "sd_op_gemm_plan: head-major K / V needs N = 3 C and a KV buffer");
        a.KV = (bf16_t*)KV; a.hm_C = N / 3; a.hm_tok = hm_tokens;
    }
    return sd_launch_gemm(a, 0, (hipStream_t)stream);
}
extern "C" int sd_op_gemm_ln(void* stream, const void* X, long long ldx, const void* Wg, const float* c1, const float* c2,
                             const float* rowstats, int parts, float eps, void* C, long long ldc, int M, int N, int K, int epi) {
    if (ensure_zero_page()) return -2;
    SD_REQUIRE(epi == 0 || epi == 1, "sd_op_gemm_ln: epi %d (0 = plain, 1 = GEGLU)", epi);
    GemmArgs a;
    a.X = (const bf16_t*)X; a.ldx = ldx; a.K1 = K; a.W = (const bf16_t*)Wg; a.bias = c2;
    a.C = (bf16_t*)C; a.ldc = ldc; a.M = M; a.N = N; a.K = K; a.zero_page = zero_page(); a.splitk = 1;
    a.ln_rs = rowstats; a.ln_np = parts; a.ln_c1 = c1; a.ln_eps = eps;
    return sd_launch_gemm(a, epi, (hipStream_t)stream);
}

extern "C" int sd_op_xattn_fused_rowstats(void* stream, const void* X, const void* R, void* Y, const void* At, const void* Bw,
                                          const float* bias, int M, int C, int rows_per_sample, int L, float* rowstats) {
    SD_REQUIRE(sd_xattn_fused_applicable(rows_per_sample, C, 8, L), "sd_op_xattn_fused_rowstats: shape not supported");
    XattnArgs a = xattn_args(X, R, Y, At, Bw, bias, M, C, rows_per_sample, L);
    a.rowstats = rowstats;
    return sd_launch_xattn_fused(a, (hipStream_t)stream);
}

extern "C" int sd_op_ip_xattn(void* stream, const void* R, void* Rout, const void* A, const void* Bt, const float* gamma,
                              const float* beta, float eps, long long M, int C, int rows_per_sample, int heads, int T) {
    return sd_launch_ip_xattn((const bf16_t*)R, (bf16_t*)Rout, (const bf16_t*)A, (const bf16_t*)Bt, gamma, beta, eps, (long)M, C,
                              rows_per_sample, heads, T, (hipStream_t)stream);
}

extern "C" int sd_op_xattn_fused(void* stream, const void* X, const void* R, void* Y, const void* At, const void* Bw,
                                 const float* bias, int M, int C, int rows_per_sample, int L) {
    SD_REQUIRE(sd_xattn_fused_applicable(rows_per_sample, C, 8, L) || getenv("SD_XATTN_FUSED"),
               "sd_op_xattn_fused: shape not supported (8 heads x 80 key slots, 64 < L <= 80, C %% 32 == 0, tokens per sample %% 128 == 0)");
    return sd_launch_xattn_fused(xattn_args(X, R, Y, At, Bw, bias, M, C, rows_per_sample, L), (hipStream_t)stream);
}

extern "C" int sd_op_xattn_fused_ln(void* stream, const void* X, const void* R, void* Y, const void* At, const void* Bw,
                                    const float* bias, int M, int C, int rows_per_sample, int L, const float* ln_rowstats,
                                    int ln_parts, long long ln_rows, const float* c2, float eps, float* rowstats) {
    SD_REQUIRE(sd_xattn_fused_applicable(rows_per_sample, C, 8, L), "sd_op_xattn_fused_ln: shape not supported");
    SD_REQUIRE(ln_rowstats && c2, "sd_op_xattn_fused_ln: null operand");
    XattnArgs a = xattn_args(X, R, Y, At, Bw, bias, M, C, rows_per_sample, L);
    a.rowstats = rowstats;
    a.ln_rs = ln_rowstats; a.ln_np = ln_parts; a.ln_rows = ln_rows; a.ln_c2 = c2; a.ln_eps = eps;
    return sd_launch_xattn_fused(a, (hipStream_t)stream);
}

extern "C" int sd_op_xattn_fused_stamps(void* stream, const void* X, const void* R, void* Y, const void* At, const void* Bw,
                                        const float* bias, int M, int C, int rows_per_sample, int L, unsigned long long* stamps) {
    SD_REQUIRE(stamps, "sd_op_xattn_fused_stamps: null stamp buffer");
    SD_REQUIRE(sd_xattn_fused_applicable(rows_per_sample, C, 8, L), "sd_op_xattn_fused_stamps: shape not supported");
    XattnArgs a = xattn_args(X, R, Y, At, Bw, bias, M, C, rows_per_sample, L);
    a.stamps = stamps;
    return sd_launch_xattn_fused(a, (hipStream_t)stream);
}
```

sonicdiffusionbayeslab_amd/csrc/plan.hip:

```cpp
#include "model.h"

#include <stdlib.h>

namespace sdhip {

namespace {

struct Builder {
    sd_unet* u;
    Plan& pl;
    int UB;
    std::vector<Wrap> wrapstack;
    std::map<int, int> stats_of;
    std::map<int, float> tscale;
    static std::string stem(const std::string& key) {
        const size_t n = key.rfind(".weight");
        return n == std::string::npos ? key : key.substr(0, n);
    }
    std::string error;
    float xscale(int t) {
        auto it = tscale.find(t);
        if (it == tscale.end()) {
            if (error.empty()) error = "fp8 consumer of a tensor without a scale";
            return 1.0f;
        }
        return it->second;
    }
    bool producer_stats = !(getenv("SD_GN_PRODUCER_STATS") && atoi(getenv("SD_GN_PRODUCER_STATS")) == 0);
    void want_stats(Op& o, int M, int N) {
        if (!producer_stats || !u->unet_like() || o.splitk > 1 || M % 64 != 0 || o.epi != 0 || o.rpb != 0) return;
        o.stats = tensor((size_t)(M / 64) * N * 2 * 4);
        stats_of[o.out] = o.stats;
    }

    int prefix_rep = 1;
    int replicate(int t, size_t bytes, int r) {
        Op o; o.kind = OP_REPLICATE; o.x1 = t; o.M = (int)(bytes / 16); o.N = r; o.out = tensor(bytes * r);
        push(o);
        return o.out;
    }
    bool ln_fold = !(getenv("SD_LN_FOLD") && atoi(getenv("SD_LN_FOLD")) == 0);
    int want_rowstats(Op& o, int M, int C, int& rs) {
        int np = 0;
        if (o.kind == OP_GEMM && o.epi == 0 && o.splitk == 1 && !o.out_fp8 && o.N == C && o.M == M && o.ldc_o == 0) np = (C + 159) / 160 * 2;
        else if (o.kind == OP_XATTN && o.N == C && o.M == M) np = 2 * sd_xattn_slices(M, C);
        static const bool big_tiles = getenv("SD_GEMM_BIG") != nullptr;
        if (!ln_fold || np == 0 || np > 16 || C < 128 || big_tiles) return 0;
        o.rs = rs = tensor((size_t)np * M * 2 * 4);
        return np;
    }
    int gemm_ln(int x, int rs, int np, int M, int N, int C, const std::string& w, int epi) {
        Op o; o.kind = OP_GEMM; o.x1 = x; o.K1 = o.K = o.Kalg = C; o.M = M; o.N = N; o.epi = epi; o.splitk = 1;
        o.w = W(w + ".ln"); o.c1 = W(w + ".c1"); o.b = W(w + ".c2"); o.lnrs = rs; o.lnnp = np;
        o.out = tensor((size_t)M * (epi ? N / 2 : N) * 2);
        push(o);
        return o.out;
    }

    int ctx_tensor(size_t bytes) {
        const int id = tensor(bytes, true);
        pl.tensors[id].ctx = true;
        return id;
    }
    int ctx_ip_tensor(size_t bytes) {
        const int id = ctx_tensor(bytes);
        pl.tensors[id].ctx_ip = true;
        return id;
    }
    int tensor(size_t bytes, bool persistent = false) {
        Tn t;
        t.bytes = (bytes + 255) / 256 * 256;
        t.persistent = persistent;
        pl.tensors.push_back(t);
        return (int)pl.tensors.size() - 1;
    }
    size_t W(const std::string& k) {
        auto it = u->woff.find(k);
        if (it == u->woff.end()) {
            if (error.empty()) error = "missing packed weight " + k;
            return 0;
        }
        return it->second;
    }
    Op& push(Op op) {
        op.nwrap = (int)wrapstack.size();
        for (int i = 0; i < op.nwrap; ++i) op.wraps[i] = wrapstack[i];
        pl.ops.push_back(op);
        return pl.ops.back();
    }
    static int pad128(int c) { return (c + 127) / 128 * 128; }
    int gn(int x1, int c1, int x2, int c2, int hw, const std::string& g, const std::string& b, float eps, int silu,
           bool fq = false) {
        Op o; o.kind = OP_GN; o.x1 = x1; o.C1 = c1; o.x2 = x2; o.C2 = c2; o.HW = hw; o.B = UB;
        o.g = W(g); o.be = W(b); o.eps = eps; o.silu = silu;
        o.nsplit = sd_groupnorm_nsplit(UB, hw);
        o.aux = tensor(sd_groupnorm_scratch_bytes(UB, hw, u->cfg.norm_num_groups));
        if (hw % 64 == 0 && !sd_groupnorm_uses_small(UB, hw, c1, c2, u->cfg.norm_num_groups) && stats_of.count(x1) &&
            (x2 < 0 || stats_of.count(x2))) {
            o.s1 = stats_of[x1];
            o.s2 = x2 >= 0 ? stats_of[x2] : -1;
        }
        if (fq) {
            o.out_fp8 = 1; o.Cpad = pad128(c1 + c2); o.sname = u->act_id(stem(g), u->s_norm); o.os = u->act_scale[o.sname];
            o.out = tensor((size_t)UB * hw * o.Cpad); tscale[o.out] = o.os;
        } else o.out = tensor((size_t)UB * hw * (c1 + c2) * 2);
        push(o);
        return o.out;
    }
    int conv3(int x, int hin, int win, int cin, int cout, int stride, int up, const std::string& w, const std::string& b,
              long b2idx, int b2t, int r, bool fq = false) {
        Op o; o.kind = OP_CONV3; o.x1 = x; o.B = UB; o.Hin = hin; o.Win = win; o.Cin = cin; o.N = cout;
        o.stride = stride; o.up = up;
        o.Hout = ((hin << up) + 2 - 3) / stride + 1;
        o.Wout = ((win << up) + 2 - 3) / stride + 1;
        o.M = UB * o.Hout * o.Wout; o.K = 9 * cin; o.Kalg = o.K;
        o.b = W(b); o.b2t = b2t; o.b2idx = b2idx; o.r = r;
        if (fq) { o.dt = 1; o.Cin = pad128(cin); o.K = 9 * o.Cin; o.w = W(w + ".fp8"); o.wsc = W(w + ".scale"); o.xs = xscale(x); }
        else o.w = W(w);
        static const bool subpix_off = getenv("SD_CONV_SUBPIXEL") && atoi(getenv("SD_CONV_SUBPIXEL")) == 0;
        if (up && !fq && !subpix_off && u->kind == 0 && stride == 1 && r < 0 && b2t < 0 && (hin * win) % 64 == 0 &&
            u->woff.count(w + ".sub")) {
            o.subpix = 1; o.K = 4 * cin; o.Kalg = 4 * cin;
            o.w = W(w + ".sub"); o.splitk = 1;
            o.out = tensor((size_t)o.M * cout * 2);
            if ((hin * win) % 128 == 0) want_stats(o, o.M, cout);
            push(o);
            return o.out;
        }
        o.splitk = sd_conv3x3_splitk(o.M, o.N, o.Cin, hin, win, stride, up, o.dt);
        if (o.splitk > 1) o.aux = tensor((size_t)o.splitk * o.M * o.N * 4);
        o.out = tensor((size_t)o.M * cout * 2);
        GemmArgs g;
        g.M = o.M; g.N = o.N; g.Cin = o.Cin; g.K = o.K; g.ldw = o.K; g.Hin = hin; g.Win = win; g.Hout = o.Hout; g.Wout = o.Wout;
        g.stride = stride; g.up = up; g.dt = o.dt;
        if (sd_conv_halo_mode(g) != 2) want_stats(o, o.M, cout);
        push(o);
        return o.out;
    }
    int gemm(int x1, int k1, int x2, int k2, int M, int N, const std::string& w, const std::string& b, int r, int epi,
             bool fq = false, const std::string& oname = "") {
        Op o; o.kind = OP_GEMM; o.x1 = x1; o.x2 = x2; o.K1 = k1; o.K = k1 + k2; o.Kalg = o.K; o.M = M; o.N = N; o.epi = epi;
        o.b = b.empty() ? NOFF : W(b); o.r = r;
        if (fq) { o.dt = 1; o.K = o.K1 = pad128(k1); o.w = W(w + ".fp8"); o.wsc = W(w + ".scale"); o.xs = xscale(x1); }
        else o.w = W(w);
        o.splitk = epi ? 1 : sd_gemm_splitk(M, N, o.dt ? o.K / 2 : o.K, o.dt ? 128 : 0);
        if (o.splitk > 1) o.aux = tensor((size_t)o.splitk * M * N * 4);
        if (!oname.empty()) {
            o.out_fp8 = 1; o.sname = u->act_id(oname, u->s_ff); o.os = u->act_scale[o.sname]; o.Cpad = pad128(N / 2);
            o.out = tensor((size_t)M * o.Cpad); tscale[o.out] = o.os;
        } else o.out = tensor((size_t)M * (epi ? N / 2 : N) * 2);
        push(o);
        return o.out;
    }
    int ln(int x, int M, int C, const std::string& g, const std::string& b, bool fq = false, float eps = 1e-5f) {
        Op o; o.kind = OP_LN; o.x1 = x; o.M = M; o.N = C; o.g = W(g); o.be = W(b); o.eps = eps;
        if (fq) {
            o.out_fp8 = 1; o.Cpad = pad128(C); o.sname = u->act_id(stem(g), u->s_norm); o.os = u->act_scale[o.sname];
            o.out = tensor((size_t)M * o.Cpad); tscale[o.out] = o.os;
        } else o.out = tensor((size_t)M * C * 2);
        push(o);
        return o.out;
    }
    int attn(int q, long qoff, long ldq, int kv, long koff, long voff, long ldkv, int nq, int nk, int C, int heads) {
        Op o; o.kind = OP_ATTN; o.x1 = q; o.x2 = kv; o.qoff = qoff; o.koff = koff; o.voff = voff;
        o.ldq = ldq; o.ldk = o.ldv = ldkv; o.ldo = C; o.B = UB; o.heads = heads; o.D = C / heads;
        o.Nq = nq; o.Nk = nk;
        o.out = tensor((size_t)UB * nq * C * 2);
        push(o);
        return o.out;
    }
    bool shortcut_fuse = !(getenv("SD_SHORTCUT_FUSE") && atoi(getenv("SD_SHORTCUT_FUSE")) == 0);
    int resnet(const std::string& p, int x1, int c1, int x2, int c2, int cout, int rh, int rw, int tproj_t) {
        const int hw = rh * rw, cin = c1 + c2, M = UB * hw;
        const bool fq = u->fp8;
        int t1 = gn(x1, c1, x2, c2, hw, p + "norm1.weight", p + "norm1.bias", u->cfg.norm_eps, 1, fq);
        int t2 = conv3(t1, rh, rw, cin, cout, 1, 0, p + "conv1.weight", p + "conv1.bias", u->tproj_off.at(p), tproj_t, -1, fq);
        int t3 = gn(t2, cout, -1, 0, hw, p + "norm2.weight", p + "norm2.bias", u->cfg.norm_eps, 1, fq);
        int sc = x1;
        if (cin != cout) {
            GemmArgs g;
            g.M = M; g.N = cout; g.Cin = cout; g.K = 9 * cout; g.ldw = g.K; g.Hin = g.Hout = rh; g.Win = g.Wout = rw;
            g.Csc1 = c1; g.Csc2 = x2 >= 0 ? c2 : 0;
            if (shortcut_fuse && !fq && u->unet_like() && u->woff.count(p + "conv2.bias+shortcut") && sd_conv_halo_shortcut_applicable(g)) {
                const int out = conv3(t3, rh, rw, cout, cout, 1, 0, p + "conv2.weight", p + "conv2.bias+shortcut", 0, -1, -1, fq);
                Op& o = pl.ops.back();
                o.scx1 = x1; o.scc1 = c1; o.scx2 = x2; o.scc2 = g.Csc2; o.scw = W(p + "conv_shortcut.weight");
                o.Kalg += cin;
                return out;
            }
            sc = gemm(x1, c1, x2, c2, M, cout, p + "conv_shortcut.weight", p + "conv_shortcut.bias", -1, 0);
        }
        return conv3(t3, rh, rw, cout, cout, 1, 0, p + "conv2.weight", p + "conv2.bias", 0, -1, sc, fq);
    }
    int tome_r(int rh, int rw, int C) {
        if (u->kind != 0 || u->fp8 || !(u->tome_ratio > 0.0) || rh <= 0 || pl.lh / rh > u->tome_max_downsample) return 0;
        const int N = rh * rw;
        if (rh % 2 || rw % 2 || N > 16384 || C % 64 || C > 1536) {
            if (error.empty()) error = "Token Merging needs even token-grid sides, at most 16384 tokens and C a multiple of 64 up to 1536 on "
                                       "every merging level (" + std::to_string(rh) + "x" + std::to_string(rw) + ", C = " + std::to_string(C) + ")";
            return 0;
        }
        return std::min(N - N / 4, (int)((double)N * u->tome_ratio));
    }
    int n_transformers = 0;
    int transformer(const std::string& p, int x, int C, int rh, int rw) {
        const int hw = rh * rw, L = u->cfg.context_len;
        const int NH = block_heads(u->cfg, p), NP = NH * 80;
        int M = UB * hw;
        const std::string t = p + "transformer_blocks.0.";
        const bool fq = u->fp8;
        int g = gn(x, C, -1, 0, hw, p + "norm.weight", p + "norm.bias", 1e-6f, 0, fq);
        int h0 = gemm(g, C, -1, 0, M, C, p + "proj_in.weight", p + "proj_in.bias", -1, 0, fq);
        const int tr = tome_r(rh, rw, C);
        const int Nm = hw - tr, Mm = UB * Nm;
        int tome_i = -1;
        int qkv, rs = -1, np = 0;
        if (tr > 0) {
            const int num_dst = hw / 4, num_src = hw - num_dst;
            Plan::TomeBlock tb;
            tb.B = UB; tb.h = rh; tb.w = rw; tb.r = tr; tb.choice_off = pl.tome_choice_bytes;
            pl.tome_choice_bytes += num_dst;
            tb.tok = tensor((size_t)hw * 4, true);
            tb.kept = tensor((size_t)UB * std::max(num_src - tr, 1) * 4, true);
            tb.merged = tensor((size_t)UB * tr * 4, true);
            tb.dst_idx = tensor((size_t)UB * tr * 4, true);
            int n1 = ln(h0, M, C, t + "norm1.weight", t + "norm1.bias");
            int nmax, nidx;
            { Op o; o.kind = OP_TOME_MATCH; o.x1 = h0; o.B = UB; o.Hin = rh; o.Win = rw; o.N = C; o.b2idx = tb.choice_off;
              o.out = nmax = tensor((size_t)UB * num_src * 4); o.aux = nidx = tensor((size_t)UB * num_src * 4);
              o.stats = tb.tok; o.rs = tensor((size_t)UB * hw * 4); push(o); }
            { Op o; o.kind = OP_TOME_SELECT; o.x1 = nmax; o.x2 = nidx; o.B = UB; o.M = num_src; o.K = tr;
              o.out = tb.kept; o.aux = tb.merged; o.stats = tb.dst_idx; push(o); }
            int m;
            { Op o; o.kind = OP_TOME_MERGE; o.x1 = n1; o.x2 = tb.tok; o.r = tb.kept; o.wt = tb.merged; o.s1 = tb.dst_idx;
              o.B = UB; o.Hin = rh; o.Win = rw; o.N = C; o.K = tr; o.out = m = tensor((size_t)Mm * C * 2); push(o); }
            tome_i = (int)pl.tome.size();
            pl.tome.push_back(tb);
            qkv = gemm(m, C, -1, 0, Mm, 3 * C, t + "attn1.qkv.weight", "", -1, 0);
        } else if (!fq && (np = want_rowstats(pl.ops.back(), M, C, rs)) > 0) {
            qkv = gemm_ln(h0, rs, np, M, 3 * C, C, t + "attn1.qkv.weight", 0);
        } else {
            int n1 = ln(h0, M, C, t + "norm1.weight", t + "norm1.bias", fq);
            qkv = gemm(n1, C, -1, 0, M, 3 * C, t + "attn1.qkv.weight", "", -1, 0, fq);
        }
        static const bool hm_off = (getenv("SD_ATTN_HEADMAJOR") && atoi(getenv("SD_ATTN_HEADMAJOR")) == 0) ||
                                   getenv("SD_ATTN_NO_PIPE") || getenv("SD_ATTN_NO_DMA") || getenv("SD_GEMM_BIG");
        const bool hm = !hm_off && C / NH == 40 && C % 160 == 0 && Nm % 128 == 0 && Nm >= 256 &&
                        sd_gemm_tile_rows(Mm, 3 * C) == 128 && pl.ops.back().splitk == 1;
        int a1;
        if (hm) {
            pl.ops.back().hm = 1;
            pl.ops.back().HW = Nm;
            a1 = attn(qkv, 0, C, qkv, (long)Mm * C, 2l * Mm * C, C, Nm, Nm, C, NH);
            pl.ops.back().hm = 1;
        } else {
            a1 = attn(qkv, 0, 3 * C, qkv, C, 2 * C, 3 * C, Nm, Nm, C, NH);
        }
        pl.ops.back().qps = 1;
        int h1 = gemm(a1, C, -1, 0, Mm, C, t + "attn1.to_out.0.weight", t + "attn1.to_out.0.bias", tr > 0 ? -1 : h0, 0);
        const int to_out_op = (int)pl.ops.size() - 1;
        if (tr > 0) {
            const Plan::TomeBlock& tb = pl.tome[tome_i];
            Op o; o.kind = OP_TOME_UNMERGE; o.x1 = h1; o.r = h0; o.x2 = tb.tok; o.wt = tb.kept; o.s1 = tb.merged; o.s2 = tb.dst_idx;
            o.B = UB; o.Hin = rh; o.Win = rw; o.N = C; o.K = tr; o.out = tensor((size_t)M * C * 2); push(o);
            h1 = o.out;
        }
        if (prefix_rep > 1) {
            x = replicate(x, (size_t)M * C * 2, prefix_rep);
            h1 = replicate(h1, (size_t)M * C * 2, prefix_rep);
            UB *= prefix_rep;
            M = UB * hw;
            prefix_rep = 1;
        }
        static const int fused_min_hw = getenv("SD_XATTN_FUSED") ? atoi(getenv("SD_XATTN_FUSED")) : 1024;
        static const int fold_max_hw = getenv("SD_XATTN_FOLD") ? atoi(getenv("SD_XATTN_FOLD")) : 1024;
        static const bool xln_off = getenv("SD_XATTN_LN") && atoi(getenv("SD_XATTN_LN")) == 0;
        const int xmode = (fused_min_hw > 0 && hw >= fused_min_hw && sd_xattn_fused_applicable(hw, C, NH, L)) ? 0
                          : (hw <= fold_max_hw && hw % 128 == 0 && L <= 80 && NP % 64 == 0) ? 1 : 2;
        int rs2 = -1, np2 = 0;
        const long rs2_rows = (long)pl.ops[to_out_op].M;
        const bool first_tf = n_transformers++ == 0;
        if (!fq && !xln_off && tr == 0 && (xmode == 0 || (!first_tf && rs2_rows == M)) &&
            u->woff.count(t + (xmode == 2 ? "attn2.to_q.weight.ln" : "attn2.to_q.weight.T.ln"))) {
            if (first_tf) pl.ops[to_out_op].splitk = 1;
            np2 = want_rowstats(pl.ops[to_out_op], (int)rs2_rows, C, rs2);
        }
        int n2 = np2 > 0 ? h1 : ln(h1, M, C, t + "norm2.weight", t + "norm2.bias");
        int kv = ctx_tensor((size_t)UB * L * 2 * C * 2);
        pl.ctx_kv.push_back(kv);
        pl.ctx_w.push_back(W(t + "attn2.kv.weight"));
        pl.ctx_c.push_back(C);
        int res = h1;
        if (pl.ip) {
            const int at = ctx_ip_tensor((size_t)UB * 32 * C * 2), bt = ctx_ip_tensor((size_t)UB * C * 32 * 2);
            pl.ip_fold.push_back(Plan::IpFold{at, bt, C, W(t + "attn2.to_q.weight.T"), W(t + "attn2.to_out.0.weight"), W(t + "attn2.kv_ip.weight"), NH});
            Op o; o.kind = OP_IP_XATTN; o.x1 = h1; o.wt = at; o.x2 = bt; o.M = M; o.N = C; o.rpb = hw; o.heads = NH;
            o.g = W(t + "norm2.weight"); o.be = W(t + "norm2.bias"); o.eps = 1e-5f;
            o.out = tensor((size_t)M * C * 2); push(o); res = o.out;
        }
        int h2;
        if (xmode == 0) {
            int at = ctx_tensor((size_t)UB * NP * C * 2), bw = ctx_tensor((size_t)UB * C * NP * 2);
            Plan::Fold fd{kv, at, bw, C, NH, W(t + (np2 > 0 ? "attn2.to_q.weight.T.ln" : "attn2.to_q.weight.T")), W(t + "attn2.to_out.0.weight"), true};
            if (np2 > 0) { fd.c2 = ctx_tensor((size_t)UB * NP * 4); fd.lnu = W(t + "attn2.to_q.lnu"); }
            pl.ctx_fold.push_back(fd);
            Op o; o.kind = OP_XATTN; o.x1 = n2; o.r = res; o.wt = at; o.x2 = bw; o.M = M; o.N = C; o.K = NP; o.rpb = hw;
            o.sm_valid = L; o.b = W(t + "attn2.to_out.0.bias"); o.heads = NH;
            if (np2 > 0) { o.lnrs = rs2; o.lnnp = np2; o.s1 = fd.c2; o.ldx_o = rs2_rows; }
            o.out = tensor((size_t)M * C * 2); push(o); h2 = o.out;
        } else if (xmode == 1) {
            int at = ctx_tensor((size_t)UB * NP * C * 2), bw = ctx_tensor((size_t)UB * C * NP * 2);
            Plan::Fold fd{kv, at, bw, C, NH, W(t + (np2 > 0 ? "attn2.to_q.weight.T.ln" : "attn2.to_q.weight.T")), W(t + "attn2.to_out.0.weight"), false};
            if (np2 > 0) {
                fd.c2 = ctx_tensor((size_t)UB * NP * 4); fd.lnu = W(t + "attn2.to_q.lnu");
                fd.c1 = ctx_tensor((size_t)UB * NP * 4); fd.ones = W(t + "attn2.to_q.ones");
            }
            pl.ctx_fold.push_back(fd);
            int pr;
            { Op o; o.kind = OP_GEMM; o.x1 = n2; o.K1 = C; o.K = C; o.M = M; o.N = NP; o.epi = 2; o.sm_valid = L;
              o.wt = at; o.wbs = (long)NP * C; o.rpb = hw;
              if (np2 > 0) { o.lnrs = rs2; o.lnnp = np2; o.s1 = fd.c1; o.s2 = fd.c2; }
              o.out = tensor((size_t)M * NP * 2); push(o); pr = o.out; }
            { Op o; o.kind = OP_GEMM; o.x1 = pr; o.K1 = NP; o.K = NP; o.M = M; o.N = C; o.epi = 0;
              o.wt = bw; o.wbs = (long)C * NP; o.rpb = hw; o.b = W(t + "attn2.to_out.0.bias"); o.r = res;
              o.out = tensor((size_t)M * C * 2); push(o); h2 = o.out; }
        } else {
            int q2 = np2 > 0 ? gemm_ln(h1, rs2, np2, M, C, C, t + "attn2.to_q.weight", 0)
                             : gemm(n2, C, -1, 0, M, C, t + "attn2.to_q.weight", "", -1, 0);
            int a2 = attn(q2, 0, C, kv, 0, C, 2 * C, hw, L, C, NH);
            h2 = gemm(a2, C, -1, 0, M, C, t + "attn2.to_out.0.weight", t + "attn2.to_out.0.bias", res, 0);
        }
        int ff;
        if (!fq && (np = want_rowstats(pl.ops.back(), M, C, rs)) > 0) {
            ff = gemm_ln(h2, rs, np, M, 8 * C, C, t + "ff.geglu.weight", 1);
        } else {
            int n3 = ln(h2, M, C, t + "norm3.weight", t + "norm3.bias", fq);
            ff = gemm(n3, C, -1, 0, M, 8 * C, t + "ff.geglu.weight", t + "ff.geglu.bias", -1, 1, fq, fq ? t + "ff.net.0" : std::string());
        }
        static const bool merge_off = getenv("SD_FF_MERGE") && atoi(getenv("SD_FF_MERGE")) == 0;
        int out;
        if (!fq && !merge_off) {
            out = gemm(ff, 4 * C, h2, C, M, C, p + "ff_out.weight", p + "ff_out.bias", x, 0);
        } else {
            int h3 = gemm(ff, 4 * C, -1, 0, M, C, t + "ff.net.2.weight", t + "ff.net.2.bias", h2, 0, fq);
            out = gemm(h3, C, -1, 0, M, C, p + "proj_out.weight", p + "proj_out.bias", x, 0);
        }
        if (pl.ops.back().splitk == 1 && sd_gemm_tile_rows(M, C, pl.ops.back().K) == 128) want_stats(pl.ops.back(), M, C);
        return out;
    }

    int vae_resnet(const std::string& p, int x, int cin, int cout, int rh, int rw) {
        const int hw = rh * rw, M = UB * hw;
        int t1 = gn(x, cin, -1, 0, hw, p + "norm1.weight", p + "norm1.bias", 1e-6f, 1);
        int t2 = conv3(t1, rh, rw, cin, cout, 1, 0, p + "conv1.weight", p + "conv1.bias", 0, -1, -1);
        int t3 = gn(t2, cout, -1, 0, hw, p + "norm2.weight", p + "norm2.bias", 1e-6f, 1);
        int sc = x;
        if (cin != cout) sc = gemm(x, cin, -1, 0, M, cout, p + "conv_shortcut.weight", p + "conv_shortcut.bias", -1, 0);
        return conv3(t3, rh, rw, cout, cout, 1, 0, p + "conv2.weight", p + "conv2.bias", 0, -1, sc);
    }
    int vae_attention(const std::string& p, int x, int C, int rh, int rw) {
        const int hw = rh * rw, M = UB * hw;
        const int qc = hw <= 4096 ? hw : 2048;
        int g = gn(x, C, -1, 0, hw, p + "group_norm.weight", p + "group_norm.bias", 1e-6f, 0);
        int qk = gemm(g, C, -1, 0, M, 2 * C, p + "qk.weight", p + "qk.bias", -1, 0);
        const int vT = tensor((size_t)UB * C * hw * 2), S = tensor((size_t)qc * hw * 2), O = tensor((size_t)M * C * 2);
        for (int img = 0; img < UB; ++img) {
            {
                Op o; o.kind = OP_GEMM; o.wx = W(p + "to_v.weight"); o.ldx_o = C; o.K1 = C; o.K = C; o.M = C; o.N = hw;
                o.wt = g; o.woff_el = (long)img * hw * C; o.ldw_o = C;
                o.out = vT; o.coff = (long)img * C * hw; o.ldc_o = hw;
                push(o);
            }
            for (int q0 = 0; q0 < hw; q0 += qc) {
                const int rows = std::min(qc, hw - q0);
                {
                    Op o; o.kind = OP_GEMM; o.x1 = qk; o.xoff = ((long)img * hw + q0) * 2 * C; o.ldx_o = 2 * C; o.K1 = C; o.K = C;
                    o.M = rows; o.N = hw; o.wt = qk; o.woff_el = (long)img * hw * 2 * C + C; o.ldw_o = 2 * C;
                    o.out = S; o.ldc_o = hw;
                    push(o);
                }
                { Op o; o.kind = OP_SOFTMAX; o.x1 = S; o.out = S; o.M = rows; o.N = hw; o.scale = 1.0f / sqrtf((float)C); push(o); }
                {
                    Op o; o.kind = OP_GEMM; o.x1 = S; o.ldx_o = hw; o.K1 = hw; o.K = hw; o.M = rows; o.N = C;
                    o.wt = vT; o.woff_el = (long)img * C * hw; o.ldw_o = hw; o.b = W(p + "to_v.bias");
                    o.out = O; o.coff = ((long)img * hw + q0) * C; o.ldc_o = C;
                    push(o);
                }
            }
        }
        return gemm(O, C, -1, 0, M, C, p + "to_out.0.weight", p + "to_out.0.bias", x, 0);
    }
    void build_vae() {
        const sd_unet_config& c = u->cfg;
        const int nl = c.num_levels, top = c.block_out_channels[nl - 1];
        int rh = pl.lh, rw = pl.lw;
        int t_pq = tensor((size_t)UB * c.in_channels * rh * rw * 4);
        { Op o; o.kind = OP_PQCONV; o.x1 = T_LATENTS; o.out = t_pq; o.B = UB; o.HW = rh * rw;
          o.w = W("post_quant_conv.weight"); o.b = W("post_quant_conv.bias"); push(o); }
        int h;
        { Op o; o.kind = OP_CONV_IN; o.x1 = t_pq; o.B = UB; o.Hin = rh; o.Win = rw; o.Cin = c.in_channels; o.N = top;
          o.w = W("decoder.conv_in.weight"); o.b = W("decoder.conv_in.bias"); o.out = tensor((size_t)UB * rh * rw * top * 2);
          push(o); h = o.out; }
        pl.taps["conv_in"] = h;
        h = vae_resnet("decoder.mid_block.resnets.0.", h, top, top, rh, rw);
        h = vae_attention("decoder.mid_block.attentions.0.", h, top, rh, rw);
        h = vae_resnet("decoder.mid_block.resnets.1.", h, top, top, rh, rw);
        pl.taps["mid"] = h;
        int ch = top;
        for (int i = 0; i < nl; ++i) {
            const int co = c.block_out_channels[nl - 1 - i];
            const std::string bp = "decoder.up_blocks." + std::to_string(i) + ".";
            for (int j = 0; j < c.layers_per_block + 1; ++j) {
                h = vae_resnet(bp + "resnets." + std::to_string(j) + ".", h, ch, co, rh, rw);
                ch = co;
            }
            if (i < nl - 1) {
                h = conv3(h, rh, rw, co, co, 1, 1, bp + "upsamplers.0.conv.weight", bp + "upsamplers.0.conv.bias", 0, -1, -1);
                rh *= 2; rw *= 2;
            }
            pl.taps["up" + std::to_string(i)] = h;
        }
        int g = gn(h, ch, -1, 0, rh * rw, "decoder.conv_norm_out.weight", "decoder.conv_norm_out.bias", 1e-6f, 1);
        { Op o; o.kind = OP_CONV_OUT; o.x1 = g; o.out = T_EPS; o.B = UB; o.Hin = rh; o.Win = rw; o.Cin = ch; o.N = c.out_channels;
          o.w = W("decoder.conv_out.weight"); o.b = W("decoder.conv_out.bias"); push(o); }
    }

    void build_vae_encoder() {
        const sd_unet_config& c = u->cfg;
        const int nl = c.num_levels, top = c.block_out_channels[nl - 1], c0 = c.block_out_channels[0];
        int rh = pl.lh << (nl - 1), rw = pl.lw << (nl - 1);
// ... 504 lines not shown
```

sonicdiffusionbayeslab_amd/csrc/unet.hip:

```cpp
#include "model.h"

#include <stdarg.h>
#include <stdio.h>
#include <stdlib.h>

#include <chrono>

static thread_local char g_err[1024] = "";
void sd_set_error(const char* fmt, ...) {
    va_list ap;
    va_start(ap, fmt);
    vsnprintf(g_err, sizeof(g_err), fmt, ap);
    va_end(ap);
}
extern "C" const char* sd_last_error(void) { return g_err; }
extern "C" int sd_abi_version(void) { return 3; }

static void* g_zero_page = nullptr;

namespace sdhip {

int ensure_zero_page() {
    if (g_zero_page) return 0;
    SD_CHECK_HIP(hipMalloc(&g_zero_page, 4096));
// ... 5 lines not shown
const void* zero_page() { return g_zero_page; }

int run_op(sd_unet* u, const Plan& pl, const Op& o, char* ws, const float* latents, int latent_batch, float* eps_out,
           float timestep, hipStream_t stream) {
    auto T = [&](int id) -> char* { return id >= 0 ? ws + pl.tensors[id].off : id == T_EPS ? (char*)eps_out : nullptr; };
    const char* wb = u->dweights;
    switch (o.kind) {
        case OP_SINUSOID:
            if (u->cond_set) return sd_launch_timestep_sinusoid_row(timestep, u->dcond, (float*)T(o.out), o.N, stream);
            return sd_launch_timestep_sinusoid(timestep, (float*)T(o.out), o.N, stream);
        case OP_GEMV:
            return sd_launch_gemv((const float*)T(o.x1), (const bf16_t*)(wb + o.w), (const float*)(wb + o.b),
                                  (float*)T(o.out), o.N, o.K, o.silu_in, stream);
        case OP_CONV_IN:
            if (u->kind == 0 && o.Cin == 9) {
                SD_REQUIRE(u->inpaint_b > 0, "forward: this UNet has in_channels = 9 and no inpainting condition is set "
                                             "(sd_unet_set_inpaint_cond_hw: mask and masked-image latents)");
                SD_REQUIRE(u->inpaint_h == o.Hin && u->inpaint_w == o.Win && o.B % u->inpaint_b == 0,
                           "forward: the inpainting condition was set for batch %d at %dx%d, the forward runs batch %d at %dx%d",
                           u->inpaint_b, u->inpaint_h, u->inpaint_w, o.B, o.Hin, o.Win);
                return sd_launch_conv_in_cond(latents, latent_batch, u->dinpaint, u->inpaint_b, (const float*)(wb + o.w),
                                              (const float*)(wb + o.b), (bf16_t*)T(o.out), o.B, o.Hin, o.Win, o.N, stream);
            }
            if (u->kind == 5) {
                SD_REQUIRE(u->cn_b > 0, "controlnet_forward: no conditioning image is set (sd_controlnet_set_cond_hw)");
                SD_REQUIRE(u->cn_h == o.Hin && u->cn_w == o.Win && o.B % u->cn_b == 0,
                           "controlnet_forward: the conditioning image was set for batch %d at %dx%d, the forward runs batch %d at %dx%d",
                           u->cn_b, u->cn_h, u->cn_w, o.B, o.Hin, o.Win);
                return sd_launch_conv_in_add(latents, latent_batch, u->cn_embed, u->cn_b, (const float*)(wb + o.w),
                                             (const float*)(wb + o.b), (bf16_t*)T(o.out), o.B, o.Hin, o.Win, o.N, stream);
            }
            return sd_launch_conv_in(o.x1 >= 0 ? (const float*)T(o.x1) : latents, o.x1 >= 0 ? o.B : latent_batch,
                                     (const float*)(wb + o.w), (const float*)(wb + o.b), (bf16_t*)T(o.out), o.B, o.Hin,
                                     o.Win, o.Cin, o.N, stream);
        case OP_PQCONV:
            return sd_launch_pqconv(latents, (const float*)(wb + o.w), (const float*)(wb + o.b), (float*)T(o.out), o.B,
                                    o.HW, timestep , stream);
        case OP_SOFTMAX:
            if (o.N > 4096) return sd_launch_softmax_rows_long((bf16_t*)T(o.x1), o.M, o.N, o.scale, stream);
            return sd_launch_softmax_rows((bf16_t*)T(o.x1), o.M, o.N, o.scale, stream);
        case OP_GN: {
            GroupNormArgs a;
            a.x1 = (const bf16_t*)T(o.x1); a.C1 = o.C1; a.x2 = (const bf16_t*)T(o.x2); a.C2 = o.C2;
            a.gamma = (const float*)(wb + o.g); a.beta = (const float*)(wb + o.be);
            a.y = (bf16_t*)T(o.out); a.partial = (float*)T(o.aux);
            a.B = o.B; a.HW = o.HW; a.groups = u->cfg.norm_num_groups; a.nsplit = o.nsplit; a.eps = o.eps; a.silu = o.silu;
            a.out_fp8 = o.out_fp8; a.Cpad = o.Cpad; a.oscale = o.os;
            a.stats1 = (const float*)T(o.s1); a.stats2 = (const float*)T(o.s2);
            if (o.slab_t >= 0) {
                a.slab = (const float*)T(o.slab_t); a.splitk = o.slab_k; a.x1w = (bf16_t*)T(o.x1);
                a.sbias = o.slab_b != NOFF ? (const float*)(wb + o.slab_b) : nullptr;
                a.sbias2 = o.slab_b2t >= 0 ? (const float*)T(o.slab_b2t) + o.slab_b2idx : nullptr;
                a.sR = (const bf16_t*)T(o.slab_r); a.sldr = o.C1;
            }
            return sd_launch_groupnorm(a, stream);
        }
        case OP_CONV3: {
            GemmArgs a;
            a.X = (const bf16_t*)T(o.x1); a.W = (const bf16_t*)(wb + o.w); a.bias = (const float*)(wb + o.b);
            a.bias2 = o.b2t >= 0 ? (const float*)T(o.b2t) + o.b2idx : nullptr;
            a.R = (const bf16_t*)T(o.r); a.ldr = o.N; a.C = (bf16_t*)T(o.out); a.ldc = o.N;
            a.M = o.M; a.N = o.N; a.K = o.K; a.K1 = o.K;
            a.Hin = o.Hin; a.Win = o.Win; a.Cin = o.Cin; a.Hout = o.Hout; a.Wout = o.Wout; a.stride = o.stride; a.up = o.up;
            a.zero_page = g_zero_page; a.splitk = o.splitk; a.slab = (float*)T(o.aux); a.defer_reduce = o.defer;
            if (o.dt) { a.dt = 1; a.wscale = (const float*)(wb + o.wsc); a.xscale_inv = 1.0f / o.xs; }
            a.stats = (float*)T(o.stats);
            a.asym = o.asym;
            if (o.subpix) { a.subpix = 1; a.up = 0; a.w_batch_stride = (long)o.N * 4 * o.Cin; }
            if (o.scw != NOFF) {
                a.Xs1 = (const bf16_t*)T(o.scx1); a.Csc1 = o.scc1; a.Xs2 = (const bf16_t*)T(o.scx2); a.Csc2 = o.scc2;
                a.Wsc = (const bf16_t*)(wb + o.scw); a.ldwsc = o.scc1 + o.scc2;
            }
            return sd_launch_conv3x3(a, stream);
        }
        case OP_GEMM: {
            GemmArgs a;
            a.X = o.wx != NOFF ? (const bf16_t*)(wb + o.wx) : (const bf16_t*)T(o.x1) + o.xoff;
            a.ldx = o.ldx_o ? o.ldx_o : o.K1; a.X2 = (const bf16_t*)T(o.x2); a.ldx2 = o.K - o.K1; a.K1 = o.K1;
            a.W = o.wt >= 0 ? (const bf16_t*)T(o.wt) + o.woff_el : (const bf16_t*)(wb + o.w); a.ldw = o.ldw_o;
            a.bias = o.b != NOFF ? (const float*)(wb + o.b) : nullptr;
            a.R = (const bf16_t*)T(o.r); a.ldr = o.N; a.C = (bf16_t*)T(o.out) + o.coff;
            a.ldc = o.ldc_o ? o.ldc_o : (o.epi == 1 ? o.N / 2 : o.N);
            a.M = o.M; a.N = o.N; a.K = o.K; a.zero_page = g_zero_page; a.splitk = o.splitk; a.slab = (float*)T(o.aux);
            a.defer_reduce = o.defer;
            a.w_batch_stride = o.wbs; a.rows_per_batch = o.rpb; a.sm_valid = o.sm_valid;
            if (o.dt) { a.dt = 1; a.wscale = (const float*)(wb + o.wsc); a.xscale_inv = 1.0f / o.xs; }
            if (o.out_fp8) { a.out_fp8 = 1; a.oscale = o.os; a.ldc = o.Cpad; }
            a.stats = (float*)T(o.stats);
            a.rowstats = (float*)T(o.rs);
            if (o.hm) { a.hm_C = o.N / 3; a.hm_tok = o.HW; a.ldc = a.hm_C; a.KV = (bf16_t*)T(o.out) + (long)o.M * a.hm_C; }
            if (o.lnrs >= 0) { a.ln_rs = (const float*)T(o.lnrs); a.ln_np = o.lnnp; a.ln_c1 = (const float*)(wb + o.c1); a.ln_eps = 1e-5f; }
            if (o.lnrs >= 0 && o.s1 >= 0) { a.ln_c1 = (const float*)T(o.s1); a.bias = (const float*)T(o.s2); a.ln_per_sample = 1; }
            return sd_launch_gemm(a, o.epi, stream);
        }
        case OP_LN:
            if (o.out_fp8)
                return sd_launch_layernorm_fp8((const bf16_t*)T(o.x1), (const float*)(wb + o.g), (const float*)(wb + o.be),
                                               T(o.out), o.M, o.N, o.Cpad, o.eps, o.os, stream);
            return sd_launch_layernorm((const bf16_t*)T(o.x1), (const float*)(wb + o.g), (const float*)(wb + o.be),
                                       (bf16_t*)T(o.out), o.M, o.N, o.eps, stream);
        case OP_ATTN: {
            AttnArgs a;
            a.Q = (const bf16_t*)T(o.x1) + o.qoff; a.ldq = o.ldq;
            a.K = (const bf16_t*)T(o.x2) + o.koff; a.ldk = o.ldk;
            a.V = (const bf16_t*)T(o.x2) + o.voff; a.ldv = o.ldv;
            a.O = (bf16_t*)T(o.out); a.ldo = o.ldo;
            a.B = o.B; a.heads = o.heads; a.Nq = o.Nq; a.Nk = o.Nk; a.D = o.D;
            a.scale = 1.0f / sqrtf((float)o.D);
            a.q_prescaled = o.qps;
            a.consts = g_zero_page;
            a.kv_head_major = o.hm;
            return sd_launch_attention(a, stream);
        }
        case OP_XATTN: {
            XattnArgs a;
            a.X = (const bf16_t*)T(o.x1); a.R = (const bf16_t*)T(o.r); a.Y = (bf16_t*)T(o.out);
            a.At = (const bf16_t*)T(o.wt); a.Bw = (const bf16_t*)T(o.x2); a.bias = (const float*)(wb + o.b);
            a.M = o.M; a.C = o.N; a.rows_per_sample = o.rpb; a.L = o.sm_valid;
            a.rowstats = (float*)T(o.rs);
            if (o.lnrs >= 0) {
                a.ln_rs = (const float*)T(o.lnrs); a.ln_np = o.lnnp; a.ln_rows = o.ldx_o; a.ln_c2 = (const float*)T(o.s1); a.ln_eps = 1e-5f;
            }
            return sd_launch_xattn_fused(a, stream);
        }
        case OP_IP_XATTN:
            return sd_launch_ip_xattn((const bf16_t*)T(o.x1), (bf16_t*)T(o.out), (const bf16_t*)T(o.wt), (const bf16_t*)T(o.x2),
                                      (const float*)(wb + o.g), (const float*)(wb + o.be), o.eps, o.M, o.N, o.rpb, o.heads,
                                      u->cfg.ip_adapter_tokens, stream);
        case OP_RES_ADD: {
            SD_REQUIRE(u->ctrl_res && o.nres == (int)pl.cn_off.size() && o.nres <= MAX_CONTROL_RES, "forward: no ControlNet residuals are set");
            bf16_t* x[MAX_CONTROL_RES];
            const bf16_t* r[MAX_CONTROL_RES];
            long n[MAX_CONTROL_RES];
            for (int k = 0; k < o.nres; ++k) {
                x[k] = (bf16_t*)T(o.res_t[k]); r[k] = (const bf16_t*)(u->ctrl_res + pl.cn_off[k]); n[k] = pl.cn_count[k];
                SD_REQUIRE((size_t)n[k] * 2 <= pl.tensors[o.res_t[k]].bytes, "forward: ControlNet residual %d exceeds its tensor", k);
            }
            return sd_launch_residual_add(x, r, n, o.nres, u->ctrl_scale, stream);
        }
        case OP_REPLICATE:
            return sd_launch_replicate(T(o.x1), T(o.out), (long)o.M * 16, o.N, stream);
        case OP_TOME_MATCH:
            SD_REQUIRE(u->tome_choice && o.b2idx + (long)(o.Hin / 2) * (o.Win / 2) <= u->tome_choice_n, "forward: no Token Merging choice array");
            return sd_launch_tome_match((const bf16_t*)T(o.x1), u->tome_choice + o.b2idx, o.B, o.Hin, o.Win, o.N, (float*)T(o.out),
                                        (int*)T(o.aux), (int*)T(o.stats), (float*)T(o.rs), stream);
        case OP_TOME_SELECT:
            return sd_launch_tome_select((const float*)T(o.x1), (const int*)T(o.x2), o.B, o.M, o.K, (int*)T(o.out), (int*)T(o.aux),
                                         (int*)T(o.stats), stream);
        case OP_TOME_MERGE:
            return sd_launch_tome_merge((const bf16_t*)T(o.x1), (const int*)T(o.x2), (const int*)T(o.r), (const int*)T(o.wt),
                                        (const int*)T(o.s1), (bf16_t*)T(o.out), o.N, o.B, o.Hin, o.Win, o.N, o.K, stream);
        case OP_TOME_UNMERGE:
            return sd_launch_tome_unmerge((const bf16_t*)T(o.x1), o.N, (const bf16_t*)T(o.r), (const int*)T(o.x2), (const int*)T(o.wt),
                                          (const int*)T(o.s1), (const int*)T(o.s2), (bf16_t*)T(o.out), o.B, o.Hin, o.Win, o.N, o.K, stream);
        case OP_CLIP_EMBED:
            if (u->kind == 6)
                return sd_launch_clip_embed(u->ir_ids, (const bf16_t*)(wb + o.w), (const bf16_t*)(wb + o.g), (bf16_t*)T(o.out),
                                            o.M, o.Nk, o.N, u->ir.vocab_size, stream);
            return sd_launch_clip_embed((const int*)latents, (const bf16_t*)(wb + o.w), (const bf16_t*)(wb + o.g),
                                        (bf16_t*)T(o.out), o.M, o.Nk, o.N, u->clip.vocab_size, stream);
        case OP_BERT_ATTN:
            return sd_launch_bert_attention((const bf16_t*)T(o.x1) + o.qoff, o.ldq, (const bf16_t*)T(o.x2) + o.koff,
                                            (const bf16_t*)T(o.x2) + o.voff, o.ldk, o.key_mask ? u->ir_mask : nullptr,
                                            (bf16_t*)T(o.out), o.ldo, o.B, o.heads, o.Nq, o.Nk, stream);
        case OP_REWARD_HEAD:
            return sd_launch_reward_head((const bf16_t*)T(o.x1), (long)o.Nq * o.N, (const float*)(wb + o.w), (const float*)(wb + o.b),
                                         u->ir.reward_mean, u->ir.reward_std, o.B, o.N, eps_out, u->ir_features, stream);
// ... 1073 lines not shown
    SD_REQUIRE((long long)pl->total_bytes <= workspace_bytes, "forward_profiled: workspace too small");
    hipStream_t st = (hipStream_t)stream;
    std::vector<hipEvent_t> ev;
    std::vector<int> which;
    auto mark = [&]() -> int {
        hipEvent_t e;
        SD_CHECK_HIP(hipEventCreate(&e));
        SD_CHECK_HIP(hipEventRecord(e, st));
        ev.push_back(e);
        return 0;
    };
    if (mark()) return -2;
    for (size_t i = 0; i < pl->ops.size(); ++i) {
        if (cache_mode == SD_CACHE_SKIP && pl->skipped[i]) continue;
        rc = run_op(u, *pl, pl->ops[i], (char*)workspace, latents, latent_batch, eps_out, timestep, st);
        if (mark()) return -2;
        which.push_back((int)i);
        if (rc) break;
    }
    SD_CHECK_HIP(hipStreamSynchronize(st));
    for (size_t j = 0; j < which.size(); ++j) {
        float ms = 0.f;
        (void)hipEventElapsedTime(&ms, ev[j], ev[j + 1]);
        per_op->push_back({which[j], ms});
    }
    for (auto e : ev) (void)hipEventDestroy(e);
    return rc;
}

extern "C" int sd_unet_forward_profiled(sd_unet* u, void* stream, const float* latents, int latent_batch, int unet_batch,
                                        float timestep, float* eps_out, void* workspace, long long workspace_bytes,
                                        int cache_mode, int cache_branch_id, double kind_ms[SD_PROFILE_KINDS],
                                        long long kind_launches[SD_PROFILE_KINDS], double kind_flops[SD_PROFILE_KINDS],
                                        double kind_bytes[SD_PROFILE_KINDS]) {
    SD_REQUIRE(kind_ms && kind_launches && kind_flops && kind_bytes, "forward_profiled: null argument");
    Plan* pl = nullptr;
    std::vector<std::pair<int, float>> per_op;
    const int rc = profiled_run(u, stream, latents, latent_batch, unet_batch, timestep, eps_out, workspace, workspace_bytes,
                                cache_mode, cache_branch_id, &pl, &per_op);
    if (!pl) return rc;
    for (int k = 0; k < SD_PROFILE_KINDS; ++k) { kind_ms[k] = 0; kind_launches[k] = 0; kind_flops[k] = 0; kind_bytes[k] = 0; }
    for (auto& [i, ms] : per_op) {
        const Op& o = pl->ops[i];
        double fl, by;
        op_work(o, &fl, &by);
        bool halo4 = false;
        if (o.kind == OP_CONV3 && !o.dt && o.subpix) {
            GemmArgs a;
            a.M = o.M; a.N = o.N; a.K = o.K; a.K1 = o.K; a.Hin = o.Hin; a.Win = o.Win; a.Cin = o.Cin; a.Hout = o.Hout; a.Wout = o.Wout;
            a.stride = o.stride; a.up = 0; a.subpix = 1; a.splitk = o.splitk; a.slab = (float*)(o.aux >= 0 ? (void*)1 : nullptr);
            a.w_batch_stride = (long)o.N * 4 * o.Cin;
            halo4 = sd_conv_halo_subpix_applicable(a);
        }
        const int kd = o.kind == OP_XATTN ? 18 : o.kind == OP_REPLICATE ? 19 : o.kind == OP_IP_XATTN ? 22 : o.kind == OP_RES_ADD ? 23 : halo4 ? 21 :
                       (o.kind == OP_CONV3 && !o.dt && (o.subpix || o.stride != 1)) ? 20 :
                       (o.dt ? (o.kind == OP_CONV3 ? 16 : 17) : o.kind);
        kind_ms[kd] += ms; kind_launches[kd] += 1; kind_flops[kd] += fl; kind_bytes[kd] += by;
    }
    return rc;
}

extern "C" long long sd_unet_forward_op_times(sd_unet* u, void* stream, const float* latents, int latent_batch, int unet_batch,
                                              float timestep, float* eps_out, void* workspace, long long workspace_bytes,
                                              int cache_mode, int cache_branch_id, char* text, long long cap) {
    SD_REQUIRE(text && cap > 0, "forward_op_times: null argument");
    Plan* pl = nullptr;
    std::vector<std::pair<int, float>> per_op;
    const int rc = profiled_run(u, stream, latents, latent_batch, unet_batch, timestep, eps_out, workspace, workspace_bytes,
                                cache_mode, cache_branch_id, &pl, &per_op);
    if (rc) return rc;
    long long n = 0;
    for (auto& [i, ms] : per_op) {
        const Op& o = pl->ops[i];
        double fl, by;
        op_work(o, &fl, &by);
        const int w = snprintf(text + n, (size_t)(cap - n), "%d %d %d %d %d %.5f %.3f %.3f\n", i, (int)o.kind, o.M, o.N,
                               o.kind == OP_GN ? o.slab_k : o.K, ms, fl * 1e-9, by * 1e-6);
        if (w < 0 || n + w >= cap) break;
        n += w;
    }
    return n;
}

extern "C" int sd_unet_debug_tensor(sd_unet* u, void* stream, const char* name, float* host_out, long long numel,
                                    void* workspace, int unet_batch, int cache_branch_id) {
    SD_REQUIRE(u && u->debug_taps, "debug_tensor: create the handle with SD_DEBUG_TAPS=1 in the environment");
    if (u->kind == 5 && name && !strcmp(name, "cond_embedding")) {
        SD_REQUIRE(u->cn_b > 0, "debug_tensor: no conditioning image is set");
        const size_t have = (size_t)u->cn_b * u->cn_h * u->cn_w * u->cfg.block_out_channels[0];
        SD_REQUIRE(numel >= 0 && (size_t)numel <= have, "debug_tensor: 'cond_embedding' holds %zu elements", have);
        std::vector<unsigned short> tmp(numel);
        SD_CHECK_HIP(hipStreamSynchronize((hipStream_t)stream));
        SD_CHECK_HIP(hipMemcpy(tmp.data(), u->cn_embed, (size_t)numel * 2, hipMemcpyDeviceToHost));
        for (long long i = 0; i < numel; ++i) {
            unsigned v = (unsigned)tmp[i] << 16;
            memcpy(&host_out[i], &v, 4);
        }
        return 0;
    }
    Plan* pl;
    int rc = get_plan(u, unet_batch, cache_branch_id, &pl, u->last_rep, u->last_h > 0 ? u->last_h : -1, u->last_w > 0 ? u->last_w : -1, u->last_ip, u->last_cn);
    if (rc) return rc;
    auto it = pl->taps.find(name);
    SD_REQUIRE(it != pl->taps.end(), "debug_tensor: unknown tap '%s'", name);
    const Tn& t = pl->tensors[it->second];
    SD_REQUIRE((size_t)numel * 2 <= t.bytes, "debug_tensor: '%s' holds at most %zu elements", name, t.bytes / 2);
    std::vector<unsigned short> tmp(numel);
    SD_CHECK_HIP(hipStreamSynchronize((hipStream_t)stream));
    SD_CHECK_HIP(hipMemcpy(tmp.data(), (char*)workspace + t.off, (size_t)numel * 2, hipMemcpyDeviceToHost));
    for (long long i = 0; i < numel; ++i) {
        unsigned v = (unsigned)tmp[i] << 16;
        memcpy(&host_out[i], &v, 4);
    }
    return 0;
}

extern "C" int sd_sched_step(void* stream, const float* eps, int cfg, float guidance, const float* x, const float* m1,
                             const float* m2, const float* m3, const float* noise, float* prev, float* y2, float* m_out,
                             const float coef[10], long long n) {
    SD_REQUIRE(coef, "sched_step: null coefficients");
    StepCoef c{coef[0], coef[1], coef[2], coef[3], coef[4], coef[5], coef[6], coef[7], coef[8], coef[9]};
    return sd_launch_sched_step(eps, cfg, guidance, x, m1, m2, m3, noise, prev, y2, m_out, c, (long)n, (hipStream_t)stream);
}

extern "C" int sd_cfg_rescale_factors(void* stream, const float* eps, int batch, long long n_per_sample, float guidance,
                                      float rescale, float* k_out) {
    return sd_launch_cfg_rescale_factors(eps, batch, (long)n_per_sample, guidance, rescale, k_out, (hipStream_t)stream);
}

extern "C" int sd_sched_step_rescaled(void* stream, const float* eps, int cfg, float guidance, const float* x,
                                      const float* m1, const float* m2, const float* m3, const float* noise, float* prev,
                                      float* y2, float* m_out, const float coef[10], long long n, const float* k,
                                      long long n_per_sample) {
    SD_REQUIRE(coef, "sched_step_rescaled: null coefficients");
    StepCoef c{coef[0], coef[1], coef[2], coef[3], coef[4], coef[5], coef[6], coef[7], coef[8], coef[9]};
    return sd_launch_sched_step_rescaled(eps, cfg, guidance, x, m1, m2, m3, noise, prev, y2, m_out, c, k, (long)n_per_sample,
                                         (long)n, (hipStream_t)stream);
}

extern "C" int sd_sched_step_inpaint(void* stream, const float* eps, int cfg, float guidance, const float* x, const float* m1,
                                     const float* m2, const float* m3, const float* noise, float* prev, float* y2,
                                     float* m_out, const float coef[10], long long n, const float* k, long long n_per_sample,
                                     const float* init, const float* blend_noise, const float* mask, float a, float s,
                                     long long hw) {
    SD_REQUIRE(coef, "sched_step_inpaint: null coefficients");
    StepCoef c{coef[0], coef[1], coef[2], coef[3], coef[4], coef[5], coef[6], coef[7], coef[8], coef[9]};
    return sd_launch_sched_step_inpaint(eps, cfg, guidance, x, m1, m2, m3, noise, prev, y2, m_out, c, k, (long)n_per_sample,
                                        (long)n, init, blend_noise, mask, a, s, (long)hw, (hipStream_t)stream);
}

extern "C" int sd_inpaint_prepare(void* stream, const float* image, const float* mask, float* masked_image, float* latent_mask,
                                  int batch, int height, int width) {
    return sd_launch_inpaint_prepare(image, mask, masked_image, latent_mask, batch, height, width, (hipStream_t)stream);
}
```

Measured before the change: 11.56 images/s.

## Add intra-block sliced-K GEMM kernel for split-K-prone UNet GEMM shapes

```diff
diff --git a/include/sd_hip.h b/include/sd_hip.h
--- a/include/sd_hip.h
+++ b/include/sd_hip.h
@@ -212,6 +212,8 @@
 long long sd_unet_forward_op_times(sd_unet* u, void* stream, const float* latents, int latent_batch, int unet_batch,
                                    float timestep, float* eps_out, void* workspace, long long workspace_bytes, int cache_mode,
                                    int cache_branch_id, char* text, long long cap);
+
+long long sd_unet_plan_gemms_hw(sd_unet* u, int unet_batch, int rep, int latent_h, int latent_w, char* text, long long cap);
 
 int sd_unet_debug_tensor(sd_unet* u, void* stream, const char* name, float* host_out, long long numel,
                          void* workspace, int unet_batch, int cache_branch_id);
@@ -314,6 +316,16 @@
                     const float* bias, const float* bias2, const void* R, long long ldr, void* C, long long ldc, int M, int N,
                     int K, float* rowstats, float* stats, const float* ln_rs, int ln_parts, const float* ln_c1, float ln_eps,
                     void* KV, int hm_tokens);
+int sd_op_gemm_slicek(void* stream, const void* X, long long ldx, const void* X2, long long ldx2, int K1, const void* W,
+                      const float* bias, const float* bias2, const void* R, long long ldr, void* C, long long ldc, int M, int N,
+                      int K, float* rowstats, float* stats, const float* ln_rs, int ln_parts, const float* ln_c1, float ln_eps,
+                      void* KV, int hm_tokens);
+int sd_op_gemm_split(void* stream, const void* X, long long ldx, const void* X2, long long ldx2, int K1, const void* W,
+                     const float* bias, const float* bias2, const void* R, long long ldr, void* C, long long ldc, int M,
+                     int N, int K, int splitk);
+int sd_op_gemm_slicek_choice(int M, int N, int K);
+int sd_op_gemm_slicek_applicable(int M, int N, int K, int K1, int epi, int dtype, int rows_per_batch, int splitk, int side,
+                                 int ln_parts, int hm_tokens);
 int sd_op_xattn_fused_rowstats(void* stream, const void* X, const void* R, void* Y, const void* At, const void* Bw,
                                const float* bias, int M, int C, int rows_per_sample, int L, float* rowstats);
 int sd_op_ip_xattn(void* stream, const void* R, void* Rout, const void* A, const void* Bt, const float* gamma, const float* beta,
diff --git a/sonicdiffusionbayeslab_amd/_lib.py b/sonicdiffusionbayeslab_amd/_lib.py
--- a/sonicdiffusionbayeslab_amd/_lib.py
+++ b/sonicdiffusionbayeslab_amd/_lib.py
@@ -144,6 +144,7 @@
     "sd_op_avgpool3x3": (_i, [_vp, _vp, _vp, _i, _i, _i, _i, _i, _i]),
     "sd_op_global_mean": (_i, [_vp, _vp, _vp, _i, _i, _i]),
     "sd_op_inception_resize": (_i, [_vp, _vp, _i, _i, _i, _vp, _i]),
+    "sd_unet_plan_gemms_hw": (_ll, [_vp, _i, _i, _i, _i, C.c_char_p, _ll]),
     "sd_unet_debug_tensor": (_i, [_vp, _vp, C.c_char_p, _vp, _ll, _vp, _i, _i]),
     "sd_sched_step": (_i, [_vp, _vp, _i, _f, _vp, _vp, _vp, _vp, _vp, _vp, _vp, _vp, C.POINTER(_f), _ll]),
     "sd_cfg_rescale_factors": (_i, [_vp, _vp, _i, _ll, _f, _f, _vp]),
@@ -193,6 +194,11 @@
     "sd_op_gemm_rowstats": (_i, [_vp, _vp, _ll, _vp, _vp, _vp, _ll, _vp, _ll, _i, _i, _i, _vp]),
     "sd_op_gemm_plan": (_i, [_vp, _vp, _ll, _vp, _ll, _i, _vp, _vp, _vp, _vp, _ll, _vp, _ll, _i, _i, _i, _vp, _vp, _vp, _i, _vp, _f,
                             _vp, _i]),
+    "sd_op_gemm_slicek": (_i, [_vp, _vp, _ll, _vp, _ll, _i, _vp, _vp, _vp, _vp, _ll, _vp, _ll, _i, _i, _i, _vp, _vp, _vp, _i, _vp, _f,
+                              _vp, _i]),
+    "sd_op_gemm_split": (_i, [_vp, _vp, _ll, _vp, _ll, _i, _vp, _vp, _vp, _vp, _ll, _vp, _ll, _i, _i, _i, _i]),
+    "sd_op_gemm_slicek_choice": (_i, [_i, _i, _i]),
+    "sd_op_gemm_slicek_applicable": (_i, [_i, _i, _i, _i, _i, _i, _i, _i, _i, _i, _i]),
     "sd_op_gemm_ln": (_i, [_vp, _vp, _ll, _vp, _vp, _vp, _vp, _i, _f, _vp, _ll, _i, _i, _i, _i]),
     "sd_op_xattn_fused_rowstats": (_i, [_vp, _vp, _vp, _vp, _vp, _vp, _vp, _i, _i, _i, _i, _vp]),
     "sd_op_xattn_fused": (_i, [_vp, _vp, _vp, _vp, _vp, _vp, _vp, _i, _i, _i, _i]),
diff --git a/sonicdiffusionbayeslab_amd/csrc/gemm_conv.hip b/sonicdiffusionbayeslab_amd/csrc/gemm_conv.hip
--- a/sonicdiffusionbayeslab_amd/csrc/gemm_conv.hip
+++ b/sonicdiffusionbayeslab_amd/csrc/gemm_conv.hip
@@ -686,7 +686,7 @@
 static int check_headmajor(const GemmArgs& a, int epi) {
     if (!a.hm_C) return 0;
     SD_REQUIRE(epi == EPI_STD && a.KV && a.hm_C % 160 == 0 && a.N == 3 * a.hm_C && a.hm_tok % 128 == 0 && a.M % a.hm_tok == 0 &&
-                   !(a.splitk > 1 && a.slab) && big_tile_mode() == 0 && sd_gemm_tile_rows(a.M, a.N) == 128,
+                   !(a.splitk > 1 && a.slab) && big_tile_mode() == 0 && (a.slicek == 2 || sd_gemm_tile_rows(a.M, a.N) == 128),
                "head-major K / V: N = 3 C with C %% 160 == 0, tokens per sample %% 128 == 0, 128 x 160 tiles, no split-K");
     return 0;
 }
@@ -739,6 +739,11 @@
         return launch<128, 160, 2, 2, 2, AMODE_GEMM, EPI_SOFTMAX>(a, stream);
     }
     if (a.rows_per_batch) return launch<128, 160, 2, 2, 2, AMODE_GEMM, EPI_STD>(a, stream);
+    if (a.slicek) {
+        SD_REQUIRE(big_tile_mode() == 0 && sd_gemm_slicek_applicable(a, epi), "gemm: sliced K on a problem it does not take (M=%d N=%d K=%d epi=%d)",
+                   a.M, a.N, a.K, epi);
+        return sd_launch_gemm_lean(a, 0, 128, stream);
+    }
     if (!lean_off && big_tile_mode() == 0 && sd_gemm_lean_applicable(a, epi)) {
         const int rows = (!a.stats && !a.ln_rs && !a.hm_C) ? sd_gemm_tile_rows(a.M, a.N, a.K) : 128;
         return sd_launch_gemm_lean(a, 0, rows, stream);
diff --git a/sonicdiffusionbayeslab_amd/csrc/gemm_lean.hip b/sonicdiffusionbayeslab_amd/csrc/gemm_lean.hip
--- a/sonicdiffusionbayeslab_amd/csrc/gemm_lean.hip
+++ b/sonicdiffusionbayeslab_amd/csrc/gemm_lean.hip
@@ -360,6 +360,335 @@
     }
 }
 
+template <int NP>
+__global__ __launch_bounds__(512, 2) void gemm_lean_slicek_kernel(const LeanArgs p) {
+    constexpr bool LN = NP > 0;
+    constexpr int BM = 128, BN = 160, WAVES_M = 2, WAVES_N = 2, NW = 4;
+    constexpr int WTM = BM / WAVES_M, WTN = BN / WAVES_N, TM = WTM / 16, TN = WTN / 16;
+    constexpr int XPW = BM / 8 / NW, WPW = BN / 8 / NW;
+    constexpr int STAGE_BYTES = (BM + BN) * 128, PAIR_BYTES = 2 * STAGE_BYTES;
+    constexpr int RED_TAIL = 2 * PAIR_BYTES;
+    constexpr int RED_BYTES = BM * BN * 4;
+    static_assert(RED_BYTES > PAIR_BYTES && (RED_BYTES - PAIR_BYTES) % 1024 == 0 && PAIR_BYTES % 1024 == 0, "reduce buffer layout");
+    static_assert(TM * TN * 4 + (TM + TN) * 8 <= 200, "accumulators + two fragment sets fit 256 registers");
+
+    extern __shared__ __attribute__((aligned(16))) char smem[];
+    char* lnbuf = smem + RED_TAIL + (RED_BYTES - PAIR_BYTES);
+    char* vecs = lnbuf + NW * 512;
+
+    const int tid = threadIdx.x, lane = tid & 63;
+    const int wave8 = __builtin_amdgcn_readfirstlane(tid >> 6);
+    const int slice = wave8 >> 2, wave = wave8 & 3;
+    const int wm = wave % WAVES_M, wn = wave / WAVES_M;
+    const int lrow = lane & 15, lq = lane >> 4;
+
+    const int nblk = gridDim.x;
+    int work;
+    {
+        const int q = nblk >> 3, r = nblk & 7, xcd = blockIdx.x & 7, idx = blockIdx.x >> 3;
+        work = (xcd < r ? xcd * (q + 1) : r * (q + 1) + (xcd - r) * q) + idx;
+    }
+    const int nwork = p.tiles_m * p.tiles_n;
+    if (work >= nwork) return;
+    int tile_m = work / p.tiles_n, tile_n = work - tile_m * p.tiles_n;
+    const int dm = nblk / p.tiles_n, dn = nblk - dm * p.tiles_n;
+
+    const rsrc_t rX = make_rsrc(p.X, p.x_bytes), rW = make_rsrc(p.W, p.w_bytes), rC = make_rsrc(p.C, p.c_bytes);
+    const rsrc_t rX2 = make_rsrc(LN ? p.X : p.X2, LN ? 0 : p.x2_bytes), rR = make_rsrc(LN ? p.X : p.R, LN ? 0 : p.r_bytes);
+    const rsrc_t rKV = make_rsrc(LN ? p.KV : p.C, LN ? p.kv_bytes : 0);
+
+    const int lrow8 = lane >> 3, gch = (lane & 7) ^ lrow8;
+    const int vX = lrow8 * p.ldxb + gch * 16, vX2 = lrow8 * p.ldx2b + gch * 16, vW = lrow8 * p.ldwb + gch * 16;
+    const int rowl = wm * WTM + lrow;
+    const int vR = rowl * p.ldrb + (wn * WTN + lq * 4) * 2;
+    const int vCw = rowl * p.ldcb + (wn * WTN + (lq & 1) * 16 + (lq >> 1) * 8) * 2;
+    const int vCn = rowl * p.ldcb + (wn * WTN + lq * 4) * 2;
+    int vH[TN / 2 + 1] = {};
+#pragma unroll
+    for (int j = 0; LN && j <= TN / 2; ++j) {
+        const int cl = wn * WTN + (j < TN / 2 ? j * 32 + (lq & 1) * 16 + (lq >> 1) * 8 : (TN - 1) * 16 + lq * 4);
+        const int hl = (cl * 205) >> 13;
+        vH[j] = ((hl << p.hm_tok_shift) + rowl) * 80 + (cl - hl * 40) * 2;
+    }
+    const int vLn = (wm * WTM + lane) * 8;
+    const int vRs = rowl * 8;
+    const int vSt = (wn * WTN + lq * 4) * 8;
+    const int vVec = (wn * WTN + lane * 4) * 4;
+
+    const int swz[2] = {((lq) ^ (lane & 7)) << 4, ((4 + lq) ^ (lane & 7)) << 4};
+    const int xoff = (wm * WTM + lrow) * 128;
+    const int woff = BM * 128 + (wn * WTN + lrow) * 128;
+
+    const int KT = p.K >> 6;
+    const int kb = slice ? KT >> 1 : 0;
+    const int nk = slice ? KT - (KT >> 1) : KT >> 1;
+    const int NI = KT - (KT >> 1);
+    int m0 = tile_m * BM, n0 = tile_n * BN;
+
+    auto stage = [&](int i, int buf) {
+        char* xs = smem + buf * PAIR_BYTES + slice * STAGE_BYTES;
+        char* ws = xs + BM * 128;
+        const int k0 = (kb + (i < nk ? i : nk - 1)) * 64;
+        if (LN || k0 < p.K1) {
+            const int so = (m0 + wave * 8) * p.ldxb + k0 * 2;
+#pragma unroll
+            for (int i2 = 0; i2 < XPW; ++i2) dma16(rX, xs + (wave + i2 * NW) * 1024, vX, so + i2 * (NW * 8) * p.ldxb);
+        } else {
+            const int so = (m0 + wave * 8) * p.ldx2b + (k0 - p.K1) * 2;
+#pragma unroll
+            for (int i2 = 0; i2 < XPW; ++i2) dma16(rX2, xs + (wave + i2 * NW) * 1024, vX2, so + i2 * (NW * 8) * p.ldx2b);
+        }
+        const int sw = (n0 + wave * 8) * p.ldwb + k0 * 2;
+#pragma unroll
+        for (int i2 = 0; i2 < WPW; ++i2) dma16(rW, ws + (wave + i2 * NW) * 1024, vW, sw + i2 * (NW * 8) * p.ldwb);
+    };
+
+    f32x4 acc[TN][TM];
+    bf16x8 xf0[TM], wf0[TN], xf1[TM], wf1[TN];
+    auto load_frags = [&](const char* sb, int ks, bf16x8* xf, bf16x8* wf) {
+#pragma unroll
+        for (int t = 0; t < TM; ++t) xf[t] = *(const bf16x8*)(sb + xoff + t * 2048 + swz[ks]);
+#pragma unroll
+        for (int t = 0; t < TN; ++t) wf[t] = *(const bf16x8*)(sb + woff + t * 2048 + swz[ks]);
+    };
+    auto mfmas = [&](const bf16x8* xf, const bf16x8* wf) {
+#pragma unroll
+        for (int a = 0; a < TN; ++a)
+#pragma unroll
+            for (int b = 0; b < TM; ++b)
+                acc[a][b] = __builtin_amdgcn_mfma_f32_16x16x32_bf16(wf[a], xf[b], acc[a][b], 0, 0, 0);
+    };
+    constexpr int RED_SPLIT = (PAIR_BYTES - 3 * TN * TM * 1024) / 1024;
+    static_assert(TN * TM == 20 && RED_SPLIT == 12, "reduce buffer: wave 3 crosses into the tail at r = 12");
+    const int red_lo = wave * (TN * TM) * 1024 + lane * 16;
+    const int red_hi = wave == 3 ? RED_TAIL - PAIR_BYTES + red_lo : red_lo;
+
+    constexpr int EPI_STORES = (TN / 2 + 1) * TM;
+    int g = 0;
+    bool stores_pending = false;
+    stage(0, 0);
+    while (true) {
+#pragma unroll
+        for (int a = 0; a < TN; ++a)
+#pragma unroll
+            for (int b = 0; b < TM; ++b) acc[a][b] = f32x4{0.f, 0.f, 0.f, 0.f};
+        for (int i = 0; i < NI - 1; ++i) {
+            if (i == 0 && stores_pending) wait_vmcnt<EPI_STORES>();
+            else wait_vmcnt<0>();
+            __builtin_amdgcn_s_barrier();
+            asm volatile("" ::: "memory");
+            const char* sb = smem + ((g + i) & 1) * PAIR_BYTES + slice * STAGE_BYTES;
+            load_frags(sb, 0, xf0, wf0);
+            __builtin_amdgcn_sched_barrier(0);
+            stage(i + 1, (g + i + 1) & 1);
+            if (i == 0 && slice == 0 && wm == 0 && lane < WTN / 4) {
+                glds16((const char*)p.vec0 + (long)n0 * 4 + (unsigned)vVec, vecs + wn * WTN * 4);
+                glds16((const char*)p.vec1 + (long)n0 * 4 + (unsigned)vVec, vecs + BN * 4 + wn * WTN * 4);
+            }
+            __builtin_amdgcn_sched_barrier(0);
+            load_frags(sb, 1, xf1, wf1);
+            mfmas(xf0, wf0);
+            mfmas(xf1, wf1);
+        }
+        wait_vmcnt<0>();
+        __builtin_amdgcn_s_barrier();
+        asm volatile("" ::: "memory");
+        u32x2 ep[LN ? NP : TN * TM];
+        {
+            const char* sb = smem + ((g + NI - 1) & 1) * PAIR_BYTES + slice * STAGE_BYTES;
+            const bool real = nk == NI;
+            if (slice == 0) {
+                if (LN) {
+                    const char* src = (const char*)p.ln_rs + (long)m0 * 8;
+#pragma unroll
+                    for (int i = 0; i < NP; ++i) ep[i] = *(const u32x2*)((src + (long)i * p.M * 8) + (unsigned)vLn);
+                } else if (p.R) {
+                    const int so = m0 * p.ldrb + n0 * 2;
+#pragma unroll
+                    for (int b = 0; b < TM; ++b)
+#pragma unroll
+                        for (int a = 0; a < TN; ++a)
+                            ep[a * TM + b] = __builtin_bit_cast(u32x2, __builtin_amdgcn_raw_buffer_load_b64(rR, vR + a * 32, so + b * 16 * p.ldrb, 0));
+                }
+            }
+            __builtin_amdgcn_sched_barrier(0);
+            if (real) {
+                load_frags(sb, 0, xf0, wf0);
+                mfmas(xf0, wf0);
+                load_frags(sb, 1, xf0, wf0);
+                mfmas(xf0, wf0);
+            }
+            __builtin_amdgcn_sched_barrier(0);
+        }
+        f32x2_t mr[LN ? TM : 1];
+        if (LN && slice == 0) {
+            float s = 0.f, q = 0.f;
+#pragma unroll
+            for (int i = 0; i < NP; ++i) {
+                const f32x2_t e = __builtin_bit_cast(f32x2_t, ep[i]);
+                s += e[0];
+                q += e[1];
+            }
+            *(f32x2_t*)(lnbuf + wave * 512 + lane * 8) = ln_mean_rstd(s, q, p.inv_k, p.ln_eps);
+#pragma unroll
+            for (int b = 0; b < TM; ++b) mr[b] = *(const f32x2_t*)(lnbuf + wave * 512 + (b * 16 + lrow) * 8);
+        }
+        g += NI;
+
+        const int em0 = m0, en0 = n0, etile_n = tile_n;
+        work += nblk;
+        const bool more = work < nwork;
+        if (more) {
+            tile_n += dn; tile_m += dm;
+            if (tile_n >= p.tiles_n) { tile_n -= p.tiles_n; tile_m += 1; }
+            m0 = tile_m * BM; n0 = tile_n * BN;
+        }
+
+        __builtin_amdgcn_s_barrier();
+        asm volatile("" ::: "memory");
+        const int par = (g + 1) & 1;
+        char* const rlo = smem + par * PAIR_BYTES + red_lo;
+        char* const rhi = smem + (wave == 3 ? 0 : par * PAIR_BYTES) + red_hi;
+        if (slice == 1) {
+#pragma unroll
+            for (int a = 0; a < TN; ++a)
+#pragma unroll
+                for (int b = 0; b < TM; ++b) *(f32x4*)((a * TM + b < RED_SPLIT ? rlo : rhi) + (a * TM + b) * 1024) = acc[a][b];
+            if (more) stage(0, g & 1);
+        }
+        asm volatile("s_waitcnt lgkmcnt(0)" ::: "memory");
+        __builtin_amdgcn_s_barrier();
+        asm volatile("" ::: "memory");
+        if (slice == 1) {
+            if (!more) break;
+            continue;
+        }
+#pragma unroll
+        for (int a = 0; a < TN; ++a) {
+            f32x4 t[TM];
+#pragma unroll
+            for (int b = 0; b < TM; ++b) t[b] = *(const f32x4*)((a * TM + b < RED_SPLIT ? rlo : rhi) + (a * TM + b) * 1024);
+#pragma unroll
+            for (int b = 0; b < TM; ++b) acc[a][b] += t[b];
+            __builtin_amdgcn_sched_barrier(0);
+        }
+
+        f32x4 v0[TN], v1[TN];
+#pragma unroll
+        for (int a = 0; a < TN; ++a) {
+            v0[a] = *(const f32x4*)(vecs + (wn * WTN + a * 16 + lq * 4) * 4);
+            v1[a] = *(const f32x4*)(vecs + BN * 4 + (wn * WTN + a * 16 + lq * 4) * 4);
+        }
+        if (LN) {
+#pragma unroll
+            for (int a = 0; a < TN; ++a)
+#pragma unroll
+                for (int b = 0; b < TM; ++b) acc[a][b] = ln_fold(acc[a][b], v0[a], mr[b][0], mr[b][1], v1[a]);
+        } else {
+#pragma unroll
+            for (int a = 0; a < TN; ++a)
+#pragma unroll
+                for (int b = 0; b < TM; ++b) {
+                    acc[a][b] += v0[a];
+                    acc[a][b] += v1[a];
+                }
+            if (p.R) {
+#pragma unroll
+                for (int a = 0; a < TN; ++a)
+#pragma unroll
+                    for (int b = 0; b < TM; ++b) {
+                        const u32x2 r = ep[a * TM + b];
+                        acc[a][b][0] += bflo(r[0]); acc[a][b][1] += bfhi(r[0]);
+                        acc[a][b][2] += bflo(r[1]); acc[a][b][3] += bfhi(r[1]);
+                    }
+            }
+        }
+
+        if (more) {
+            stage(0, g & 1);
+            stores_pending = true;
+        }
+
+        if (!LN && p.stats) {
+            char* dst = (char*)p.stats + ((long)((em0 + wm * WTM) >> 6) * p.N + en0) * 8 + (unsigned)vSt;
+#pragma unroll
+            for (int a = 0; a < TN; ++a) {
+                float sv[4] = {0.f, 0.f, 0.f, 0.f}, qv[4] = {0.f, 0.f, 0.f, 0.f};
+#pragma unroll
+                for (int b = 0; b < TM; ++b) {
+                    const unsigned p0 = pack2bf(acc[a][b][0], acc[a][b][1]), p1 = pack2bf(acc[a][b][2], acc[a][b][3]);
+                    const float v[4] = {bflo(p0), bfhi(p0), bflo(p1), bfhi(p1)};
+#pragma unroll
+                    for (int j = 0; j < 4; ++j) { sv[j] += v[j]; qv[j] = __builtin_fmaf(v[j], v[j], qv[j]); }
+                }
+#pragma unroll
+                for (int j = 0; j < 4; ++j) {
+                    sv[j] = row_shr_add<8>(row_shr_add<4>(row_shr_add<2>(row_shr_add<1>(sv[j]))));
+                    qv[j] = row_shr_add<8>(row_shr_add<4>(row_shr_add<2>(row_shr_add<1>(qv[j]))));
+                }
+                if (lrow == 15) {
+                    *(f32x4*)(dst + a * 128) = f32x4{sv[0], qv[0], sv[1], qv[1]};
+                    *(f32x4*)(dst + a * 128 + 16) = f32x4{sv[2], qv[2], sv[3], qv[3]};
+                }
+            }
+        }
+        if (!LN && p.rowstats) {
+            char* dst = (char*)p.rowstats + ((long)(etile_n * WAVES_N + wn) * p.M + em0) * 8 + (unsigned)vRs;
+#pragma unroll
+            for (int b = 0; b < TM; ++b) {
+                float s = 0.f, q = 0.f;
+#pragma unroll
+                for (int a = 0; a < TN; ++a) {
+                    const unsigned p0 = pack2bf(acc[a][b][0], acc[a][b][1]), p1 = pack2bf(acc[a][b][2], acc[a][b][3]);
+                    const float v[4] = {bflo(p0), bfhi(p0), bflo(p1), bfhi(p1)};
+#pragma unroll
+                    for (int j = 0; j < 4; ++j) { s += v[j]; q = __builtin_fmaf(v[j], v[j], q); }
+                }
+                s += __shfl_xor(s, 16); q += __shfl_xor(q, 16);
+                s += __shfl_xor(s, 32); q += __shfl_xor(q, 32);
+                if (lq == 0) *(f32x2_t*)(dst + b * 16 * 8) = f32x2_t{s, q};
+            }
+        }
+        u32x4 ow[TM][TN / 2];
+        u32x2 on[TM];
+#pragma unroll
+        for (int b = 0; b < TM; ++b) {
+#pragma unroll
+            for (int a = 0; a + 1 < TN; a += 2) {
+                const f32x4 vx = acc[a][b], vy = acc[a + 1][b];
+                const auto s0 = __builtin_amdgcn_permlane16_swap(pack2bf(vx[0], vx[1]), pack2bf(vy[0], vy[1]), false, false);
+                const auto s1 = __builtin_amdgcn_permlane16_swap(pack2bf(vx[2], vx[3]), pack2bf(vy[2], vy[3]), false, false);
+                ow[b][a / 2] = u32x4{s0[0], s1[0], s0[1], s1[1]};
+            }
+            const f32x4 v = acc[TN - 1][b];
+            on[b] = u32x2{pack2bf(v[0], v[1]), pack2bf(v[2], v[3])};
+        }
+        if (LN && p.hm_tpc > 0 && etile_n >= p.hm_tpc) {
+            const int which = etile_n >= 2 * p.hm_tpc ? 1 : 0;
+            const int head0 = (etile_n - (which + 1) * p.hm_tpc) * 4;
+            const int smp = em0 >> p.hm_tok_shift, tok0 = em0 & ((1 << p.hm_tok_shift) - 1);
+            const int soC = ((((which * p.hm_samples + smp) * p.hm_heads + head0) << p.hm_tok_shift) + tok0) * 80;
+#pragma unroll
+            for (int b = 0; b < TM; ++b) {
+                const int so = soC + b * 16 * 80;
+#pragma unroll
+                for (int j = 0; j < TN / 2; ++j) __builtin_amdgcn_raw_buffer_store_b128(ow[b][j], rKV, vH[j] + so, 0, 0);
+                __builtin_amdgcn_raw_buffer_store_b64(on[b], rKV, vH[TN / 2] + so, 0, 0);
+            }
+        } else {
+            const int soC = em0 * p.ldcb + en0 * 2;
+#pragma unroll
+            for (int b = 0; b < TM; ++b) {
+                const int so = soC + b * 16 * p.ldcb;
+#pragma unroll
+                for (int j = 0; j < TN / 2; ++j) __builtin_amdgcn_raw_buffer_store_b128(ow[b][j], rC, vCw + so + j * 64, 0, 0);
+                __builtin_amdgcn_raw_buffer_store_b64(on[b], rC, vCn + so + (TN - 1) * 32, 0, 0);
+            }
+        }
+        if (!more) break;
+    }
+}
+
 static const float* zero_vector() {
     static std::mutex mu;
     static float* z[16] = {};
@@ -397,6 +726,26 @@
     constexpr int resident = smem > 80 * 1024 ? 256 : 512;
     if (grid > resident) grid = resident;
     hipLaunchKernelGGL(kern, dim3(grid), dim3(NW * 64), smem, stream, a);
+    SD_CHECK_HIP(hipGetLastError());
+    return 0;
+}
+
+template <int NP>
+int launch_slicek(const LeanArgs& a0, hipStream_t stream) {
+    LeanArgs a = a0;
+    a.tiles_m = (a.M + 127) / 128;
+    a.tiles_n = a.N / 160;
+    constexpr int smem = 4 * (128 + 160) * 128 + (128 * 160 * 4 - 2 * (128 + 160) * 128) + 4 * 512 + 2 * 160 * 4;
+    static_assert(smem <= 160 * 1024, "tile does not fit the 160 KiB LDS");
+    auto kern = gemm_lean_slicek_kernel<NP>;
+    static bool attr_set = false;
+    if (!attr_set) {
+        SD_CHECK_HIP(hipFuncSetAttribute((const void*)kern, hipFuncAttributeMaxDynamicSharedMemorySize, smem));
+        attr_set = true;
+    }
+    int grid = a.tiles_m * a.tiles_n;
+    if (grid > 256) grid = 256;
+    hipLaunchKernelGGL(kern, dim3(grid), dim3(512), smem, stream, a);
     SD_CHECK_HIP(hipGetLastError());
     return 0;
 }
@@ -428,8 +777,24 @@
     return true;
 }
 
+bool sd_gemm_slicek_applicable(const GemmArgs& a, int epi) {
+    if (epi != 0 || a.splitk > 1 || a.K < 256 || !sd_gemm_lean_applicable(a, 0)) return false;
+    if (a.ln_rs && a.ln_np != 16) return false;
+    return true;
+}
+
+bool sd_gemm_slicek_shape(int M, int N, int K) {
+    const char* env = getenv("SD_GEMM_SLICEK");
+    if (!env || atoi(env) != 1) return false;
+    if (M < 128 || M % 128 != 0 || N % 160 != 0 || K % 64 != 0 || K < 256) return false;
+    const long tiles = (long)(M / 128) * (N / 160);
+    return tiles == 256 || tiles == 3 * 256;
+}
+
 int sd_launch_gemm_lean(const GemmArgs& g, int epi, int rows, hipStream_t stream) {
     SD_REQUIRE(sd_gemm_lean_applicable(g, epi), "gemm (lean): problem not supported (M=%d N=%d K=%d epi=%d)", g.M, g.N, g.K, epi);
+    SD_REQUIRE(g.slicek == 0 || (g.slicek == 2 && rows == 128 && sd_gemm_slicek_applicable(g, epi)),
+               "gemm (lean): sliced K (%d) on a problem it does not take (M=%d N=%d K=%d epi=%d splitk=%d)", g.slicek, g.M, g.N, g.K, epi, g.splitk);
     SD_REQUIRE(epi == 1 || rows == 128 || (rows == 64 && !g.stats && !g.ln_rs && !g.hm_C),
                "gemm (lean): %d-row tile with block statistics / LayerNorm fold / head-major K|V", rows);
     const long ldw = g.ldw ? g.ldw : g.K;
@@ -467,6 +832,7 @@
              : g.ln_np == 4 ? launch_lean<256, 256, 4, 2, 4, true>(a, stream)
              : g.ln_np == 8 ? launch_lean<256, 256, 4, 2, 8, true>(a, stream) : launch_lean<256, 256, 4, 2, 16, true>(a, stream);
     }
+    if (g.slicek == 2) return g.ln_rs ? launch_slicek<16>(a, stream) : launch_slicek<0>(a, stream);
     if (g.ln_rs)
         return g.ln_np == 2 ? launch_lean<128, 160, 2, 2, 2, false>(a, stream)
              : g.ln_np == 4 ? launch_lean<128, 160, 2, 2, 4, false>(a, stream)
diff --git a/sonicdiffusionbayeslab_amd/csrc/kernels.h b/sonicdiffusionbayeslab_amd/csrc/kernels.h
--- a/sonicdiffusionbayeslab_amd/csrc/kernels.h
+++ b/sonicdiffusionbayeslab_amd/csrc/kernels.h
@@ -49,6 +49,7 @@
     const bf16_t* Wsc = nullptr;
     long ldwsc = 0;
     int Csc1 = 0, Csc2 = 0;
+    int slicek = 0;
 };
 
 int sd_gemm_tile_rows(int M, int N, int K = 0);
@@ -57,6 +58,8 @@
 int sd_launch_conv3x3(const GemmArgs& a, hipStream_t stream);
 bool sd_gemm_lean_applicable(const GemmArgs& a, int epi);
 int sd_launch_gemm_lean(const GemmArgs& a, int epi, int rows, hipStream_t stream);
+bool sd_gemm_slicek_applicable(const GemmArgs& a, int epi);
+bool sd_gemm_slicek_shape(int M, int N, int K);
 void sd_launch_splitk_reduce(const GemmArgs& a, hipStream_t stream);
 bool sd_conv_halo_applicable(const GemmArgs& a);
 int sd_conv_halo_mode(const GemmArgs& a);
diff --git a/sonicdiffusionbayeslab_amd/csrc/model.h b/sonicdiffusionbayeslab_amd/csrc/model.h
--- a/sonicdiffusionbayeslab_amd/csrc/model.h
+++ b/sonicdiffusionbayeslab_amd/csrc/model.h
@@ -59,6 +59,7 @@
     int heads = 0, D = 0, Nq = 0, Nk = 0;
     long ldq = 0, ldk = 0, ldv = 0, ldo = 0, qoff = 0, koff = 0, voff = 0;
     int silu_in = 0, splitk = 1;
+    int slicek = 0;
     int pool_by_ids = 0;
     int key_mask = 0;
     int defer = 0, slab_t = -1, slab_k = 0, slab_r = -1, slab_b2t = -1;
diff --git a/sonicdiffusionbayeslab_amd/csrc/ops.hip b/sonicdiffusionbayeslab_amd/csrc/ops.hip
--- a/sonicdiffusionbayeslab_amd/csrc/ops.hip
+++ b/sonicdiffusionbayeslab_amd/csrc/ops.hip
@@ -566,6 +566,58 @@
     }
     return sd_launch_gemm(a, 0, (hipStream_t)stream);
 }
+extern "C" int sd_op_gemm_slicek(void* stream, const void* X, long long ldx, const void* X2, long long ldx2, int K1, const void* W,
+                                 const float* bias, const float* bias2, const void* R, long long ldr, void* C, long long ldc,
+                                 int M, int N, int K, float* rowstats, float* stats, const float* ln_rs, int ln_parts,
+                                 const float* ln_c1, float ln_eps, void* KV, int hm_tokens) {
+    if (ensure_zero_page()) return -2;
+    GemmArgs a;
+    a.X = (const bf16_t*)X; a.ldx = ldx; a.X2 = (const bf16_t*)X2; a.ldx2 = ldx2; a.K1 = K1; a.W = (const bf16_t*)W;
+    a.bias = bias; a.bias2 = bias2; a.R = (const bf16_t*)R; a.ldr = ldr; a.C = (bf16_t*)C; a.ldc = ldc; a.M = M; a.N = N; a.K = K;
+    a.zero_page = zero_page(); a.splitk = 1; a.rowstats = rowstats; a.stats = stats;
+    a.ln_rs = ln_rs; a.ln_np = ln_parts; a.ln_c1 = ln_c1; a.ln_eps = ln_eps;
+    if (hm_tokens > 0) {
+        SD_REQUIRE(N % 3 == 0 && KV, "sd_op_gemm_slicek: head-major K / V needs N = 3 C and a KV buffer");
+        a.KV = (bf16_t*)KV; a.hm_C = N / 3; a.hm_tok = hm_tokens;
+    }
+    a.slicek = 2;
+    return sd_launch_gemm(a, 0, (hipStream_t)stream);
+}
+extern "C" int sd_op_gemm_split(void* stream, const void* X, long long ldx, const void* X2, long long ldx2, int K1,
+                                const void* W, const float* bias, const float* bias2, const void* R, long long ldr, void* C,
+                                long long ldc, int M, int N, int K, int splitk) {
+    if (ensure_zero_page()) return -2;
+    SD_REQUIRE(splitk >= 1 && splitk <= 8 && K / 64 >= splitk, "sd_op_gemm_split: split factor %d for %d K tiles", splitk, K / 64);
+    GemmArgs a;
+    a.X = (const bf16_t*)X; a.ldx = ldx; a.X2 = (const bf16_t*)X2; a.ldx2 = ldx2; a.K1 = K1;
+    a.W = (const bf16_t*)W; a.bias = bias; a.bias2 = bias2; a.R = (const bf16_t*)R; a.ldr = ldr;
+    a.C = (bf16_t*)C; a.ldc = ldc; a.M = M; a.N = N; a.K = K; a.zero_page = zero_page();
+    a.splitk = splitk;
+    if (splitk_slab(a, "sd_op_gemm_split")) return -1;
+    return sd_launch_gemm(a, 0, (hipStream_t)stream);
+}
+extern "C" int sd_op_gemm_slicek_choice(int M, int N, int K) {
+    SD_REQUIRE(M > 0 && N > 0 && K > 0, "gemm_slicek_choice: bad arguments");
+    return sd_gemm_slicek_shape(M, N, K) ? 1 : 0;
+}
+extern "C" int sd_op_gemm_slicek_applicable(int M, int N, int K, int K1, int epi, int dtype, int rows_per_batch, int splitk,
+                                            int side, int ln_parts, int hm_tokens) {
+    SD_REQUIRE(M > 0 && N > 0 && K > 0 && K1 > 0 && K1 <= K, "gemm_slicek_applicable: bad arguments");
+    static float dummy[4];
+    const bf16_t* pb = (const bf16_t*)dummy;
+    GemmArgs a;
+    a.X = pb; a.ldx = K1; a.K1 = K1; a.W = pb; a.C = (bf16_t*)dummy; a.ldc = N; a.M = M; a.N = N; a.K = K;
+    if (K1 < K) { a.X2 = pb; a.ldx2 = K - K1; }
+    a.bias = dummy; a.dt = dtype; a.rows_per_batch = rows_per_batch; a.splitk = splitk;
+    if (splitk > 1) a.slab = dummy;
+    if (side & 1) a.rowstats = dummy;
+    if (side & 2) a.stats = dummy;
+    if (side & 4) { a.R = pb; a.ldr = N; }
+    if (side & 8) a.bias2 = dummy;
+    if (ln_parts > 0) { a.ln_rs = dummy; a.ln_np = ln_parts; a.ln_c1 = dummy; }
+    if (hm_tokens > 0) { a.KV = (bf16_t*)dummy; a.hm_C = N / 3; a.hm_tok = hm_tokens; a.ldc = N / 3; }
+    return sd_gemm_slicek_applicable(a, epi) ? 1 : 0;
+}
 extern "C" int sd_op_gemm_ln(void* stream, const void* X, long long ldx, const void* Wg, const float* c1, const float* c2,
                              const float* rowstats, int parts, float eps, void* C, long long ldc, int M, int N, int K, int epi) {
     if (ensure_zero_page()) return -2;
diff --git a/sonicdiffusionbayeslab_amd/csrc/plan.hip b/sonicdiffusionbayeslab_amd/csrc/plan.hip
--- a/sonicdiffusionbayeslab_amd/csrc/plan.hip
+++ b/sonicdiffusionbayeslab_amd/csrc/plan.hip
@@ -52,10 +52,14 @@
     int gemm_ln(int x, int rs, int np, int M, int N, int C, const std::string& w, int epi) {
         Op o; o.kind = OP_GEMM; o.x1 = x; o.K1 = o.K = o.Kalg = C; o.M = M; o.N = N; o.epi = epi; o.splitk = 1;
         o.w = W(w + ".ln"); o.c1 = W(w + ".c1"); o.b = W(w + ".c2"); o.lnrs = rs; o.lnnp = np;
+        if (epi == 0 && np == 16 && slice_ok()) o.slicek = sd_gemm_slicek_shape(M, N, C) ? 2 : 0;
         o.out = tensor((size_t)M * (epi ? N / 2 : N) * 2);
         push(o);
         return o.out;
     }
+
+    bool in_prefix = false;
+    bool slice_ok() const { return u->unet_like() && !u->fp8 && !in_prefix; }
 
     int ctx_tensor(size_t bytes) {
         const int id = tensor(bytes, true);
@@ -138,12 +142,13 @@
         return o.out;
     }
     int gemm(int x1, int k1, int x2, int k2, int M, int N, const std::string& w, const std::string& b, int r, int epi,
-             bool fq = false, const std::string& oname = "") {
+             bool fq = false, const std::string& oname = "", bool may_slice = true) {
         Op o; o.kind = OP_GEMM; o.x1 = x1; o.x2 = x2; o.K1 = k1; o.K = k1 + k2; o.Kalg = o.K; o.M = M; o.N = N; o.epi = epi;
         o.b = b.empty() ? NOFF : W(b); o.r = r;
         if (fq) { o.dt = 1; o.K = o.K1 = pad128(k1); o.w = W(w + ".fp8"); o.wsc = W(w + ".scale"); o.xs = xscale(x1); }
         else o.w = W(w);
         o.splitk = epi ? 1 : sd_gemm_splitk(M, N, o.dt ? o.K / 2 : o.K, o.dt ? 128 : 0);
+        if (may_slice && epi == 0 && !fq && oname.empty() && slice_ok() && sd_gemm_slicek_shape(M, N, o.K)) { o.slicek = 2; o.splitk = 1; }
         if (o.splitk > 1) o.aux = tensor((size_t)o.splitk * M * N * 4);
         if (!oname.empty()) {
             o.out_fp8 = 1; o.sname = u->act_id(oname, u->s_ff); o.os = u->act_scale[o.sname]; o.Cpad = pad128(N / 2);
@@ -209,6 +214,7 @@
         int M = UB * hw;
         const std::string t = p + "transformer_blocks.0.";
         const bool fq = u->fp8;
+        in_prefix = n_transformers == 0;
         int g = gn(x, C, -1, 0, hw, p + "norm.weight", p + "norm.bias", 1e-6f, 0, fq);
         int h0 = gemm(g, C, -1, 0, M, C, p + "proj_in.weight", p + "proj_in.bias", -1, 0, fq);
         const int tr = tome_r(rh, rw, C);
@@ -236,12 +242,12 @@
               o.B = UB; o.Hin = rh; o.Win = rw; o.N = C; o.K = tr; o.out = m = tensor((size_t)Mm * C * 2); push(o); }
             tome_i = (int)pl.tome.size();
             pl.tome.push_back(tb);
-            qkv = gemm(m, C, -1, 0, Mm, 3 * C, t + "attn1.qkv.weight", "", -1, 0);
+            qkv = gemm(m, C, -1, 0, Mm, 3 * C, t + "attn1.qkv.weight", "", -1, 0, false, "", false);
         } else if (!fq && (np = want_rowstats(pl.ops.back(), M, C, rs)) > 0) {
             qkv = gemm_ln(h0, rs, np, M, 3 * C, C, t + "attn1.qkv.weight", 0);
         } else {
             int n1 = ln(h0, M, C, t + "norm1.weight", t + "norm1.bias", fq);
-            qkv = gemm(n1, C, -1, 0, M, 3 * C, t + "attn1.qkv.weight", "", -1, 0, fq);
+            qkv = gemm(n1, C, -1, 0, M, 3 * C, t + "attn1.qkv.weight", "", -1, 0, fq, "", false);
         }
         static const bool hm_off = (getenv("SD_ATTN_HEADMAJOR") && atoi(getenv("SD_ATTN_HEADMAJOR")) == 0) ||
                                    getenv("SD_ATTN_NO_PIPE") || getenv("SD_ATTN_NO_DMA") || getenv("SD_GEMM_BIG");
@@ -280,6 +286,7 @@
         int rs2 = -1, np2 = 0;
         const long rs2_rows = (long)pl.ops[to_out_op].M;
         const bool first_tf = n_transformers++ == 0;
+        in_prefix = false;
         if (!fq && !xln_off && tr == 0 && (xmode == 0 || (!first_tf && rs2_rows == M)) &&
             u->woff.count(t + (xmode == 2 ? "attn2.to_q.weight.ln" : "attn2.to_q.weight.T.ln"))) {
             if (first_tf) pl.ops[to_out_op].splitk = 1;
@@ -345,7 +352,8 @@
             int h3 = gemm(ff, 4 * C, -1, 0, M, C, t + "ff.net.2.weight", t + "ff.net.2.bias", h2, 0, fq);
             out = gemm(h3, C, -1, 0, M, C, p + "proj_out.weight", p + "proj_out.bias", x, 0);
         }
-        if (pl.ops.back().splitk == 1 && sd_gemm_tile_rows(M, C, pl.ops.back().K) == 128) want_stats(pl.ops.back(), M, C);
+        const bool was_split = pl.ops.back().slicek && sd_gemm_splitk(M, C, pl.ops.back().K) > 1;
+        if (pl.ops.back().splitk == 1 && !was_split && sd_gemm_tile_rows(M, C, pl.ops.back().K) == 128) want_stats(pl.ops.back(), M, C);
         return out;
     }
 
diff --git a/sonicdiffusionbayeslab_amd/csrc/unet.hip b/sonicdiffusionbayeslab_amd/csrc/unet.hip
--- a/sonicdiffusionbayeslab_amd/csrc/unet.hip
+++ b/sonicdiffusionbayeslab_amd/csrc/unet.hip
@@ -111,7 +111,7 @@
             a.R = (const bf16_t*)T(o.r); a.ldr = o.N; a.C = (bf16_t*)T(o.out) + o.coff;
             a.ldc = o.ldc_o ? o.ldc_o : (o.epi == 1 ? o.N / 2 : o.N);
             a.M = o.M; a.N = o.N; a.K = o.K; a.zero_page = g_zero_page; a.splitk = o.splitk; a.slab = (float*)T(o.aux);
-            a.defer_reduce = o.defer;
+            a.defer_reduce = o.defer; a.slicek = o.slicek;
             a.w_batch_stride = o.wbs; a.rows_per_batch = o.rpb; a.sm_valid = o.sm_valid;
             if (o.dt) { a.dt = 1; a.wscale = (const float*)(wb + o.wsc); a.xscale_inv = 1.0f / o.xs; }
             if (o.out_fp8) { a.out_fp8 = 1; a.oscale = o.os; a.ldc = o.Cpad; }
@@ -1351,6 +1351,22 @@
     return n;
 }
 
+extern "C" long long sd_unet_plan_gemms_hw(sd_unet* u, int unet_batch, int rep, int latent_h, int latent_w, char* text, long long cap) {
+    SD_REQUIRE(u && text && cap > 0 && (rep == 1 || rep == 2), "plan_gemms: bad argument");
+    SD_REQUIRE(rep == 1 || unet_batch % 2 == 0, "plan_gemms: the CFG-pair variant needs an even batch");
+    Plan* pl = nullptr;
+    if (get_plan(u, unet_batch, -1, &pl, rep, latent_h, latent_w)) return -1;
+    long long n = 0;
+    for (size_t i = 0; i < pl->ops.size(); ++i) {
+        const Op& o = pl->ops[i];
+        if (o.kind != OP_GEMM) continue;
+        const int w = snprintf(text + n, (size_t)(cap - n), "%zu %d %d %d %d %d %d\n", i, o.M, o.N, o.K, o.epi, o.splitk, o.slicek);
+        SD_REQUIRE(w > 0 && n + w < cap, "plan_gemms: the text buffer is too small");
+        n += w;
+    }
+    return n;
+}
+
 extern "C" int sd_unet_debug_tensor(sd_unet* u, void* stream, const char* name, float* host_out, long long numel,
                                     void* workspace, int unet_batch, int cache_branch_id) {
     SD_REQUIRE(u && u->debug_taps, "debug_tensor: create the handle with SD_DEBUG_TAPS=1 in the environment");
```

Result: no change. 11.56 images/s (-0.0%).
